# aliftffd/ViT-vs-Raw-IQ

Measured on AMD Instinct MI355X. Metric: IQ frames/sec training (fwd+loss+bwd+clip+AdamW), higher is better.
Workload: dtype bf16; 1 GPU; ViT-Tiny/16 224x224 C=1 19cls (BASELINE configs[1]); config_id=B, per_gpu_batch=256, global_batch=256, parallelism=dp1, hipgraph=True

## Files before the change

### include/iqvit.h

```cpp
#ifndef IQVIT_H
#define IQVIT_H
#include <stddef.h>
#include <stdint.h>

#ifdef __cplusplus
extern "C" {
#endif

typedef void* iq_stream_t;

enum { IQ_STATUS_OK = 0, IQ_STATUS_ARG = 1, IQ_STATUS_UNSUPPORTED = 2, IQ_STATUS_LAUNCH = 3 };

typedef struct iq_dropout {
  uint64_t seed;
  uint32_t step;
  uint32_t site;
  float p;
  const uint32_t* step_dev;
} iq_dropout_t;
#define IQ_SITE_IMPAIR 0xFFFFFFFFu
#define IQ_SITE_SYNTH 0xFFFFFFFEu

int iq_ln_supported(int D);
int iq_ln_fwd(const void* z, const float* gamma, const float* beta, void* x, float* mean, float* rstd, int M, int D,
              float eps, iq_stream_t stream);
size_t iq_ln_bwd_ws_bytes(int D);
int iq_ln_bwd(const void* dx, const void* z, const float* mean, const float* rstd, const float* gamma, void* dz,
              void* dy, const iq_dropout_t* drop, float* dgamma, float* dbeta, float* ws, int accumulate, int M,
              int D, iq_stream_t stream);
int iq_ln_bwd_partial_rows(int M, int D);

typedef struct iq_epilogue {
  const float* bias;
  int relu;
  const float* pe;
  int tok, seq, cls_off;
  iq_dropout_t drop;
  const void* gate;
  int ldg;
  float gate_scale;
  const void* residual;
  int ldr;
} iq_epilogue_t;
int iq_gemm_bf16_nt(const void* A, int lda, const void* B, int ldb, void* C, int ldc, int M, int N, int K,
                    const iq_epilogue_t* epi, iq_stream_t stream);

int iq_gemm_ln_supported(int D, int K);
int iq_gemm_bf16_ln(const void* A, int lda, const void* W, int ldw, const float* bias, const void* residual, int ldr,
                    const iq_dropout_t* drop, const float* gamma, const float* beta, float eps, void* Z, void* X,
                    float* mean, float* rstd, int M, int D, int K, iq_stream_t stream);

int iq_gemm_lnbwd_supported(int D, int K);
int iq_gemm_lnbwd_partial_rows(int M);
int iq_gemm_bf16_lnbwd(const void* A, int lda, const void* Wt, int ldw, const void* residual, int ldr, const void* z,
                       const float* mean, const float* rstd, const float* gamma, const iq_dropout_t* drop, void* dz,
                       void* dy, float* partial, int M, int D, int K, iq_stream_t stream);

int iq_ffn_chain_supported(int S, int D, int F);
int iq_ffn_chain_bwd_partial_rows(int M);
size_t iq_ffn_chain_gate_bytes(int M, int F);
int iq_ffn_chain_bwd(const void* dO, const void* W2t, const void* gate_bits, float gate_scale, void* gH, const void* W1t,
                     const void* residual, const void* z1, const float* mean, const float* rstd, const float* gamma,
                     const iq_dropout_t* drop, void* dz, void* dy, float* partial, const void* Wot, void* dA, int frames, int S,
                     int D, int F, iq_stream_t stream);
int iq_qkv_dgrad_ffn_chain_bwd(const void* gQKV, const void* Wqkv_t, const void* residual0, const void* z2, const float* mean2,
                               const float* rstd2, const float* gamma2, const iq_dropout_t* drop2, void* dz2, void* dy2, float* partial2,
                               const void* W2t, const void* gate_bits, float gate_scale, void* gH, const void* W1t, const void* residual,
                               const void* z1, const float* mean, const float* rstd, const float* gamma, const iq_dropout_t* drop, void* dz,
                               void* dy, float* partial, const void* Wot, void* dA, int frames, int S, int D, int F, iq_stream_t stream);
int iq_ffn_chain_fwd(const void* X1, const void* W1, const float* b1, const iq_dropout_t* drop1, void* H, const void* W2,
                     const float* b2, const iq_dropout_t* drop2, const float* gamma, const float* beta, float eps, void* Z,
                     void* X, float* mean, float* rstd, void* gate_bits, int frames, int S, int D, int F, iq_stream_t stream);
int iq_attn_out_ffn_chain_fwd(const void* A, const void* Wo, const float* bo, const iq_dropout_t* drop0, const void* R,
                              const float* gamma1, const float* beta1, void* Z1, void* X1, float* mean1, float* rstd1,
                              const void* W1, const float* b1, const iq_dropout_t* drop1, void* H, const void* W2, const float* b2,
                              const iq_dropout_t* drop2, const float* gamma2, const float* beta2, float eps, void* Z2, void* X,
                              float* mean2, float* rstd2, void* gate_bits, const void* Wq, const float* bq, void* Yq, int frames,
                              int S, int D, int F, iq_stream_t stream);

size_t iq_wgrad_ws_bytes(int M, int N, int K);
int iq_gemm_bf16_wgrad(const void* dY, int ldy, const void* X, int ldx, float* dW, float* dbias, int M, int N, int K,
                       float* ws, size_t ws_bytes, int accumulate, iq_stream_t stream);

typedef struct iq_wgrad_problem {
  const void* dY;
  int ldy;
  const void* X;
  int ldx;
  float* dW;
  float* dbias;
  int N, K;
} iq_wgrad_problem_t;
typedef struct iq_reduce_seg {
  const float* partials;
  int rows;
  int64_t row_stride;
  float* out;
  int64_t n;
} iq_reduce_seg_t;
size_t iq_wgrad_grouped_ws_bytes(const iq_wgrad_problem_t* probs, int nprob, int M, int max_workgroups);
int iq_gemm_bf16_wgrad_grouped(const iq_wgrad_problem_t* probs, int nprob, int M, float* ws, size_t ws_bytes,
                               int accumulate, int max_workgroups, const iq_reduce_seg_t* extra, int nextra,
                               iq_stream_t stream);

int iq_attn_supported(int S, int dh);
int iq_attn_fwd(const void* qkv, void* out, float* lse, int B, int S, int H, int dh, iq_stream_t stream);
int iq_attn_bwd(const void* qkv, const void* out, const void* dout, const float* lse, void* dqkv, int B, int S, int H,
                int dh, iq_stream_t stream);
int iq_attn_fwd_masked(const void* qkv, void* out, float* lse, const uint8_t* mask, long mask_hstride, int B, int S,
                       int H, int dh, iq_stream_t stream);
int iq_attn_bwd_masked(const void* qkv, const void* out, const void* dout, const float* lse, void* dqkv,
                       const uint8_t* mask, long mask_hstride, int B, int S, int H, int dh, iq_stream_t stream);
int iq_attn_probs(const void* qkv, const float* lse, float* out, long out_bstride, int B, int S, int H, int dh,
                  int rows, int heads, iq_stream_t stream);
int iq_attn_grad_probs(const void* qkv, const float* lse, const void* dout, float* out, long out_bstride, int B, int S,
                       int H, int dh, int rows, int heads, int positive, iq_stream_t stream);
int iq_attn_relevance_step(const void* qkv, const float* lse, const void* dout, const float* r_in, float* r_out, int B,
                           int S, int H, int dh, iq_stream_t stream);

int iq_frames_preprocess(const float* raw, float* out, int n_frames, int len, int take, const float* stats,
                         iq_stream_t stream);
typedef struct iq_impair {
  float phase_lo, phase_hi;
  float cfo_lo, cfo_hi;
  int   rot90;
  int   conj;
  int   shift_max;
  float gain_db_lo, gain_db_hi;
  float snr_db_lo, snr_db_hi;
  uint64_t seed; uint32_t step;
  uint64_t frame_base;
} iq_impair_t;
int iq_frames_impair(const float* raw, float* out, float* drawn, int n_frames, int len, int take, const float* stats,
                     const iq_impair_t* imp, iq_stream_t stream);
#define IQ_SYNTH_MAX_CLASSES 128
#define IQ_SYNTH_MAX_SNRS 64
typedef struct iq_synth_class { int kind; int offset; int count; } iq_synth_class_t;
typedef struct iq_synth {
  const float* points;
  const iq_synth_class_t* classes; int n_classes;
  const float* snrs_db; int n_snrs;
  int balanced;
  uint64_t seed; uint32_t stream;
  uint64_t frame_base;
} iq_synth_t;
int iq_frames_synth(float* raw , int64_t* labels, float* snr ,
                    float* drawn ,
                    int32_t* symbols , int n_frames, int len, const iq_synth_t* par, iq_stream_t stream);
typedef struct iq_waveform {
  const float* points; const iq_synth_class_t* classes; int n_classes;
  const float* snrs_db; int n_snrs; int balanced;
  uint64_t seed; uint32_t stream; uint64_t frame_base;
  int sps;
  int span;
  int n_phase;
  int timing;
  const float* pulse;
  const int32_t* fpulse;
  int n_taps;
  float los;
  float tap_sigma[8];
} iq_waveform_t;
int iq_frames_waveform(float* raw , int64_t* labels, float* snr, float* drawn ,
                       int32_t* symbols , float* taps , int n_frames, int len,
                       const iq_waveform_t* par, iq_stream_t stream);
enum { IQ_RX_GIVEN = 0, IQ_RX_OERDER_MEYR = 1, IQ_RX_ENERGY = 2 };
typedef struct iq_receiver {
  int sps;
  int span;
  int n_frac;
  int mode;
  int normalise;
  const float* table;
  const int32_t* u;
} iq_receiver_t;
int iq_frames_receive(const float* raw , float* sym , float* est ,
                      float* energy , int n_frames, int len, const iq_receiver_t* par, iq_stream_t stream);
int iq_frames_receive_bwd(const float* dsym , const float* sym, const float* est, float* dx ,
                          int n_frames, int len, const iq_receiver_t* par, iq_stream_t stream);
typedef struct iq_spectrogram {
  int n_fft;
  int hop;
  int pad;
  int width;
  int mode;
  float inv_norm, floor, scale, shift;
} iq_spectrogram_t;
int iq_frames_spectrogram(const float* x , const float* table ,
                          float* out , int n_frames, int len, const iq_spectrogram_t* par,
                          iq_stream_t stream);
int iq_frames_spectrogram_bwd(const float* x, const float* table, const float* dout ,
                              float* dx , int n_frames, int len, const iq_spectrogram_t* par,
                              iq_stream_t stream);
typedef struct iq_cyclic {
  int n_fft;
  int hop;
  int pad;
  int columns;
  int kind;
  int mode;
  float inv_norm, floor, scale, shift;
} iq_cyclic_t;
int iq_frames_cyclic(const float* x , const float* table , const float* rot ,
                     float* out , int n_frames, int len, const iq_cyclic_t* par, iq_stream_t stream);
int iq_patchify(const float* src, void* patches, int kind, int B, int C, int H, int W, int p, int Kpad,
                iq_stream_t stream);
int iq_cls_rows(const float* cls, const float* pe, void* x0, int B, int S, int D, const iq_dropout_t* drop,
                iq_stream_t stream);
int iq_embed_bwd_gather(const void* dx0, void* demb, float* dcls, int B, int S, int tok, int D, int has_cls,
                        const iq_dropout_t* drop, int accumulate, iq_stream_t stream);
int iq_embed_dgrad(const void* demb, const void* w_bf16, int Kpad, float* dsrc, int kind, int B, int C, int H, int W, int p,
                   int D, iq_stream_t stream);
int iq_linf_step(float* x_adv, const float* grad, const float* x0, float alpha, float eps, float lo, float hi, size_t n,
                 iq_stream_t stream);

int iq_head_fwd(const void* x, const float* ln_g, const float* ln_b, const float* W, const float* b, float* featn,
                float* hstat, float* logits, int B, int S, int D, int K, int pool, iq_stream_t stream);
int iq_ce_fwd_bwd(const float* logits, const int64_t* labels, int B, int K, float smoothing, float denom,
                  float* loss_sum, int32_t* n_correct, float* dlogits, iq_stream_t stream);
int iq_head_bwd(const float* dlogits, const float* featn, const float* hstat, const float* ln_g, const float* ln_b,
                const float* W, float* dW, float* db, float* dln_g, float* dln_b, void* dx, int B, int S, int D, int K,
                int pool, int accumulate, iq_stream_t stream);

size_t iq_gradnorm_ws_bytes(size_t n);
int iq_gradnorm_sq(const float* g, size_t n, float grad_scale, float* ws, float* out, iq_stream_t stream);
int iq_adamw_step(float* p, const float* g, float* m, float* v, void* shadow_bf16, size_t n, float lr, float beta1,
                  float beta2, float eps, float weight_decay, int step, const float* gnorm_sq, float max_norm,
                  float grad_scale, const float* dyn, iq_stream_t stream);
int iq_counter_add(uint32_t* ctr_u32, uint32_t inc_u32, float* ctr_f32, float inc_f32, iq_stream_t stream);
int iq_cast_bf16(const float* src, void* dst, size_t n, iq_stream_t stream);
int iq_transpose_cast_bf16(const float* src, void* dst, int rows, int cols, iq_stream_t stream);

typedef struct iq_model_cfg {
  int kind;
  int in_channels;
  int img_h, img_w, patch;
  int seq_length, conv_k, use_cls;
  int num_classes, d_model, n_head, n_layers, ffn_hidden;
  float drop_prob;
} iq_model_cfg_t;

typedef struct iq_model iq_model_t;

int iq_model_create(const iq_model_cfg_t* cfg, iq_model_t** out);
void iq_model_destroy(iq_model_t* m);
const char* iq_model_last_error(const iq_model_t* m);
int iq_model_tokens(const iq_model_t* m);
size_t iq_model_param_floats(const iq_model_t* m);
int iq_model_param_entries(const iq_model_t* m);
int iq_model_param_entry(const iq_model_t* m, int i, char* name, int name_cap, size_t* offset, int* ndim, int* dims);
size_t iq_model_shadow_bytes(const iq_model_t* m);
size_t iq_model_workspace_bytes(const iq_model_t* m, int batch, int training);
int iq_model_bind(iq_model_t* m, float* params, float* grads, const float* pe, void* shadow);
int iq_model_bind_step_counter(iq_model_t* m, uint32_t* counter);
int iq_model_refresh_shadow(iq_model_t* m, iq_stream_t stream);
int iq_model_refresh_transposed(iq_model_t* m, iq_stream_t stream);
int iq_model_forward(iq_model_t* m, const float* src, int batch, void* workspace, size_t ws_bytes, int training,
                     uint64_t seed, uint32_t step, float* enc_out, float* logits, iq_stream_t stream);
int iq_model_backward(iq_model_t* m, const float* dlogits, const float* denc, int batch, void* workspace,
                      size_t ws_bytes, int accumulate, int stage_hi, int stage_lo, iq_stream_t stream);
int iq_model_grad_range(const iq_model_t* m, int stage_hi, int stage_lo, size_t* off, size_t* len);
#define IQ_BWD_PARAM_GRADS 1
int iq_model_backward_input(iq_model_t* m, const float* dlogits, const float* denc, int batch, void* workspace,
                            size_t ws_bytes, float* dsrc, int flags, iq_stream_t stream);
int iq_model_attention(iq_model_t* m, const void* workspace, size_t ws_bytes, int batch, int layer, int rows,
                       int heads, float* out, long out_bstride, iq_stream_t stream);
int iq_model_attention_rollout(iq_model_t* m, const void* workspace, size_t ws_bytes, int batch, float alpha,
                               float* out, iq_stream_t stream);
int iq_model_attention_relevance(iq_model_t* m, const float* dlogits, int batch, void* workspace, size_t ws_bytes,
                                 float* rel, float* const* maps, int rows, int heads, int positive, long out_bstride,
                                 iq_stream_t stream);

#define IQ_PROF_FAMILIES 8
int iq_prof_enable(int on);
int iq_prof_collect(double* ms, long long* count);
size_t iq_prof_kernels(char* out, size_t cap, int reset);

#ifdef __cplusplus
}
#endif
#endif
```

### vit-vs-raw-iq_amd/_native.py

```python
from __future__ import annotations

import ctypes as C
import os

_HERE = os.path.dirname(os.path.abspath(__file__))
LIB_PATH = os.environ.get("IQ_LIBIQVIT") or os.path.join(_HERE, "libiqvit.so")

BWD_PARAM_GRADS = 1

STATUS = {0: "ok", 1: "invalid argument", 2: "unsupported shape/configuration", 3: "HIP launch error"}


class IqError(RuntimeError):
    pass


class Dropout(C.Structure):
    _fields_ = [("seed", C.c_uint64), ("step", C.c_uint32), ("site", C.c_uint32), ("p", C.c_float),
                ("step_dev", C.c_void_p)]


class Impair(C.Structure):
    _fields_ = [("phase_lo", C.c_float), ("phase_hi", C.c_float), ("cfo_lo", C.c_float), ("cfo_hi", C.c_float),
                ("rot90", C.c_int), ("conj", C.c_int), ("shift_max", C.c_int), ("gain_db_lo", C.c_float),
                ("gain_db_hi", C.c_float), ("snr_db_lo", C.c_float), ("snr_db_hi", C.c_float), ("seed", C.c_uint64),
                ("step", C.c_uint32), ("frame_base", C.c_uint64)]


class SynthClass(C.Structure):
    _fields_ = [("kind", C.c_int), ("offset", C.c_int), ("count", C.c_int)]


class Synth(C.Structure):
    _fields_ = [("points", C.c_void_p), ("classes", C.POINTER(SynthClass)), ("n_classes", C.c_int),
                ("snrs_db", C.POINTER(C.c_float)), ("n_snrs", C.c_int), ("balanced", C.c_int), ("seed", C.c_uint64),
                ("stream", C.c_uint32), ("frame_base", C.c_uint64)]


class Waveform(C.Structure):
    _fields_ = [("points", C.c_void_p), ("classes", C.POINTER(SynthClass)), ("n_classes", C.c_int),
                ("snrs_db", C.POINTER(C.c_float)), ("n_snrs", C.c_int), ("balanced", C.c_int), ("seed", C.c_uint64),
                ("stream", C.c_uint32), ("frame_base", C.c_uint64), ("sps", C.c_int), ("span", C.c_int), ("n_phase", C.c_int),
                ("timing", C.c_int), ("pulse", C.c_void_p), ("fpulse", C.c_void_p), ("n_taps", C.c_int), ("los", C.c_float),
                ("tap_sigma", C.c_float * 8)]


class Receiver(C.Structure):
    _fields_ = [("sps", C.c_int), ("span", C.c_int), ("n_frac", C.c_int), ("mode", C.c_int), ("normalise", C.c_int),
                ("table", C.c_void_p), ("u", C.c_void_p)]


class Spectrogram(C.Structure):
    _fields_ = [("n_fft", C.c_int), ("hop", C.c_int), ("pad", C.c_int), ("width", C.c_int), ("mode", C.c_int),
                ("inv_norm", C.c_float), ("floor", C.c_float), ("scale", C.c_float), ("shift", C.c_float)]


class Cyclic(C.Structure):
    _fields_ = [("n_fft", C.c_int), ("hop", C.c_int), ("pad", C.c_int), ("columns", C.c_int), ("kind", C.c_int),
                ("mode", C.c_int), ("inv_norm", C.c_float), ("floor", C.c_float), ("scale", C.c_float), ("shift", C.c_float)]


class Epilogue(C.Structure):
    _fields_ = [("bias", C.c_void_p), ("relu", C.c_int), ("pe", C.c_void_p), ("tok", C.c_int), ("seq", C.c_int),
                ("cls_off", C.c_int), ("drop", Dropout), ("gate", C.c_void_p), ("ldg", C.c_int),
                ("gate_scale", C.c_float), ("residual", C.c_void_p), ("ldr", C.c_int)]


class WgradProblem(C.Structure):
    _fields_ = [("dY", C.c_void_p), ("ldy", C.c_int), ("X", C.c_void_p), ("ldx", C.c_int), ("dW", C.c_void_p),
                ("dbias", C.c_void_p), ("N", C.c_int), ("K", C.c_int)]


class ReduceSeg(C.Structure):
    _fields_ = [("partials", C.c_void_p), ("rows", C.c_int), ("row_stride", C.c_int64), ("out", C.c_void_p),
                ("n", C.c_int64)]


class ModelCfg(C.Structure):
    _fields_ = [("kind", C.c_int), ("in_channels", C.c_int), ("img_h", C.c_int), ("img_w", C.c_int),
                ("patch", C.c_int), ("seq_length", C.c_int), ("conv_k", C.c_int), ("use_cls", C.c_int),
                ("num_classes", C.c_int), ("d_model", C.c_int), ("n_head", C.c_int), ("n_layers", C.c_int),
                ("ffn_hidden", C.c_int), ("drop_prob", C.c_float)]


_P, _I, _Z, _F = C.c_void_p, C.c_int, C.c_size_t, C.c_float
_U64, _U32 = C.c_uint64, C.c_uint32

SIGNATURES = {
    "iq_ln_supported": (_I, [_I]),
    "iq_ln_fwd": (_I, [_P, _P, _P, _P, _P, _P, _I, _I, _F, _P]),
    "iq_ln_bwd_ws_bytes": (_Z, [_I]),
    "iq_ln_bwd_partial_rows": (_I, [_I, _I]),
    "iq_ln_bwd": (_I, [_P, _P, _P, _P, _P, _P, _P, C.POINTER(Dropout), _P, _P, _P, _I, _I, _I, _P]),
    "iq_gemm_bf16_nt": (_I, [_P, _I, _P, _I, _P, _I, _I, _I, _I, C.POINTER(Epilogue), _P]),
    "iq_gemm_ln_supported": (_I, [_I, _I]),
    "iq_gemm_bf16_ln": (_I, [_P, _I, _P, _I, _P, _P, _I, C.POINTER(Dropout), _P, _P, _F, _P, _P, _P, _P, _I, _I, _I, _P]),
    "iq_gemm_lnbwd_supported": (_I, [_I, _I]),
    "iq_gemm_lnbwd_partial_rows": (_I, [_I]),
    "iq_gemm_bf16_lnbwd": (_I, [_P, _I, _P, _I, _P, _I, _P, _P, _P, _P, C.POINTER(Dropout), _P, _P, _P, _I, _I, _I, _P]),
    "iq_ffn_chain_supported": (_I, [_I, _I, _I]),
    "iq_ffn_chain_bwd_partial_rows": (_I, [_I]),
    "iq_ffn_chain_bwd": (_I, [_P, _P, _P, _F, _P, _P, _P, _P, _P, _P, _P, C.POINTER(Dropout), _P, _P, _P, _P, _P, _I, _I, _I, _I, _P]),
    "iq_qkv_dgrad_ffn_chain_bwd": (_I, [_P, _P, _P, _P, _P, _P, _P, C.POINTER(Dropout), _P, _P, _P,
                                        _P, _P, _F, _P, _P, _P, _P, _P, _P, _P, C.POINTER(Dropout), _P, _P, _P, _P, _P, _I, _I, _I, _I, _P]),
    "iq_ffn_chain_gate_bytes": (_Z, [_I, _I]),
    "iq_ffn_chain_fwd": (_I, [_P, _P, _P, C.POINTER(Dropout), _P, _P, _P, C.POINTER(Dropout), _P, _P, _F, _P, _P, _P, _P, _P, _I, _I,
                              _I, _I, _P]),
    "iq_attn_out_ffn_chain_fwd": (_I, [_P, _P, _P, C.POINTER(Dropout), _P, _P, _P, _P, _P, _P, _P,
                                       _P, _P, C.POINTER(Dropout), _P, _P, _P, C.POINTER(Dropout), _P, _P, _F, _P, _P, _P, _P, _P,
                                       _P, _P, _P, _I, _I, _I, _I, _P]),
    "iq_wgrad_ws_bytes": (_Z, [_I, _I, _I]),
    "iq_gemm_bf16_wgrad": (_I, [_P, _I, _P, _I, _P, _P, _I, _I, _I, _P, _Z, _I, _P]),
    "iq_wgrad_grouped_ws_bytes": (_Z, [_P, _I, _I, _I]),
    "iq_gemm_bf16_wgrad_grouped": (_I, [_P, _I, _I, _P, _Z, _I, _I, _P, _I, _P]),
    "iq_attn_supported": (_I, [_I, _I]),
    "iq_attn_fwd": (_I, [_P, _P, _P, _I, _I, _I, _I, _P]),
    "iq_attn_bwd": (_I, [_P, _P, _P, _P, _P, _I, _I, _I, _I, _P]),
    "iq_attn_fwd_masked": (_I, [_P, _P, _P, _P, C.c_long, _I, _I, _I, _I, _P]),
    "iq_attn_bwd_masked": (_I, [_P, _P, _P, _P, _P, _P, C.c_long, _I, _I, _I, _I, _P]),
    "iq_attn_probs": (_I, [_P, _P, _P, C.c_long, _I, _I, _I, _I, _I, _I, _P]),
    "iq_attn_grad_probs": (_I, [_P, _P, _P, _P, C.c_long, _I, _I, _I, _I, _I, _I, _I, _P]),
    "iq_attn_relevance_step": (_I, [_P, _P, _P, _P, _P, _I, _I, _I, _I, _P]),
    "iq_frames_preprocess": (_I, [_P, _P, _I, _I, _I, C.POINTER(C.c_float), _P]),
    "iq_frames_impair": (_I, [_P, _P, _P, _I, _I, _I, C.POINTER(C.c_float), C.POINTER(Impair), _P]),
    "iq_frames_synth": (_I, [_P, _P, _P, _P, _P, _I, _I, C.POINTER(Synth), _P]),
    "iq_frames_waveform": (_I, [_P, _P, _P, _P, _P, _P, _I, _I, C.POINTER(Waveform), _P]),
    "iq_frames_receive": (_I, [_P, _P, _P, _P, _I, _I, C.POINTER(Receiver), _P]),
    "iq_frames_receive_bwd": (_I, [_P, _P, _P, _P, _I, _I, C.POINTER(Receiver), _P]),
    "iq_frames_spectrogram": (_I, [_P, _P, _P, _I, _I, C.POINTER(Spectrogram), _P]),
    "iq_frames_spectrogram_bwd": (_I, [_P, _P, _P, _P, _I, _I, C.POINTER(Spectrogram), _P]),
    "iq_frames_cyclic": (_I, [_P, _P, _P, _P, _I, _I, C.POINTER(Cyclic), _P]),
    "iq_patchify": (_I, [_P, _P, _I, _I, _I, _I, _I, _I, _I, _P]),
    "iq_cls_rows": (_I, [_P, _P, _P, _I, _I, _I, C.POINTER(Dropout), _P]),
    "iq_embed_bwd_gather": (_I, [_P, _P, _P, _I, _I, _I, _I, _I, C.POINTER(Dropout), _I, _P]),
    "iq_embed_dgrad": (_I, [_P, _P, _I, _P, _I, _I, _I, _I, _I, _I, _I, _P]),
    "iq_linf_step": (_I, [_P, _P, _P, _F, _F, _F, _F, _Z, _P]),
    "iq_head_fwd": (_I, [_P, _P, _P, _P, _P, _P, _P, _P, _I, _I, _I, _I, _I, _P]),
    "iq_ce_fwd_bwd": (_I, [_P, _P, _I, _I, _F, _F, _P, _P, _P, _P]),
    "iq_head_bwd": (_I, [_P, _P, _P, _P, _P, _P, _P, _P, _P, _P, _P, _I, _I, _I, _I, _I, _I, _P]),
    "iq_gradnorm_ws_bytes": (_Z, [_Z]),
    "iq_gradnorm_sq": (_I, [_P, _Z, _F, _P, _P, _P]),
    "iq_adamw_step": (_I, [_P, _P, _P, _P, _P, _Z, _F, _F, _F, _F, _F, _I, _P, _F, _F, _P, _P]),
    "iq_counter_add": (_I, [_P, _U32, _P, _F, _P]),
    "iq_cast_bf16": (_I, [_P, _P, _Z, _P]),
    "iq_transpose_cast_bf16": (_I, [_P, _P, _I, _I, _P]),
    "iq_model_create": (_I, [C.POINTER(ModelCfg), C.POINTER(_P)]),
    "iq_model_destroy": (None, [_P]),
    "iq_model_last_error": (C.c_char_p, [_P]),
    "iq_model_tokens": (_I, [_P]),
    "iq_model_param_floats": (_Z, [_P]),
    "iq_model_param_entries": (_I, [_P]),
    "iq_model_param_entry": (_I, [_P, _I, C.c_char_p, _I, C.POINTER(_Z), C.POINTER(_I), C.POINTER(_I)]),
    "iq_model_shadow_bytes": (_Z, [_P]),
    "iq_model_workspace_bytes": (_Z, [_P, _I, _I]),
    "iq_model_bind": (_I, [_P, _P, _P, _P, _P]),
    "iq_model_bind_step_counter": (_I, [_P, _P]),
    "iq_model_refresh_shadow": (_I, [_P, _P]),
    "iq_model_refresh_transposed": (_I, [_P, _P]),
    "iq_model_forward": (_I, [_P, _P, _I, _P, _Z, _I, _U64, _U32, _P, _P, _P]),
    "iq_model_backward": (_I, [_P, _P, _P, _I, _P, _Z, _I, _I, _I, _P]),
    "iq_model_grad_range": (_I, [_P, _I, _I, C.POINTER(_Z), C.POINTER(_Z)]),
    "iq_model_backward_input": (_I, [_P, _P, _P, _I, _P, _Z, _P, _I, _P]),
    "iq_model_attention": (_I, [_P, _P, _Z, _I, _I, _I, _I, _P, C.c_long, _P]),
    "iq_model_attention_rollout": (_I, [_P, _P, _Z, _I, _F, _P, _P]),
    "iq_model_attention_relevance": (_I, [_P, _P, _I, _P, _Z, _P, C.POINTER(_P), _I, _I, _I, C.c_long, _P]),
    "iq_prof_enable": (_I, [_I]),
    "iq_prof_collect": (_I, [C.POINTER(C.c_double), C.POINTER(C.c_longlong)]),
    "iq_prof_kernels": (_Z, [C.c_char_p, _Z, _I]),
}

_lib = None


def lib():
    global _lib
    if _lib is None:
        if not os.path.exists(LIB_PATH):
            raise IqError(
                f"{LIB_PATH} not found: the HIP extension is not built. Run "
                "`python -c 'import __graft_entry__ as g; g.build()'` (or `make -C vit-vs-raw-iq_amd/csrc`). "
                "There is no CPU fallback.")
        L = C.CDLL(LIB_PATH)
        for name, (res, args) in SIGNATURES.items():
            fn = getattr(L, name)
            fn.restype = res
            fn.argtypes = args
        _lib = L
    return _lib


def check(rc, what, model=None):
    if rc != 0:
        detail = ""
        if model is not None:
            msg = lib().iq_model_last_error(model)
            if msg:
                detail = ": " + msg.decode()
        raise IqError(f"{what} failed: {STATUS.get(rc, rc)}{detail}")


def ptr(t):
    return None if t is None else t.data_ptr()


def stream_handle():
    import torch
    return torch.cuda.current_stream().cuda_stream
```

### vit-vs-raw-iq_amd/csrc/gemm_lnbwd.hip

```cpp

#include "common.h"
#include "gemm_common.h"
#include "gemm_ring.h"
#include "iqvit.h"
#include "prof.h"

namespace {

constexpr int LB_THREADS = 256;

struct LnBwdParams {
  const bf16* A; const bf16* B; const bf16* residual;
  int lda, ldb, ldr, M, K;
  const bf16* Z; const float* mean; const float* rstd; const float* gamma;
  bf16* dZ; bf16* dY;
  float* partial;
  int drop_on; IqRng rng; uint32_t thresh; float dscale;
};

template <int BMT, int BN>
__global__ __launch_bounds__(LB_THREADS, 2) void gemm_lnbwd_kernel(const LnBwdParams p) {
  using Ring = RingShape<BMT, BN>;
  constexpr int BK2 = Ring::BK2, NS = Ring::NS, STAGE_BYTES = Ring::STAGE_BYTES, WN = Ring::WN, NT = Ring::NT, NP = NT / 2, MT = Ring::MT;
  constexpr int A_LD = Ring::A_LD, B_LD = Ring::B_LD, PER_STAGE = Ring::PER_STAGE, NRS = Ring::NRS;
  constexpr int TAIL_LOADS = (BMT / (4 * (64 / ((BN == 192) ? 8 : 16)))) * (BN / (8 * ((BN == 192) ? 8 : 16)));
  constexpr int N = BN;
  static_assert(NRS >= 2, "tile shape");
  extern __shared__ __attribute__((aligned(16))) unsigned char smem[];

  const int tid = threadIdx.x, lane = tid & 63, wave = tid >> 6;
  const int wm = wave >> 1, wn = wave & 1;
  const int g = lane >> 4, c16 = lane & 15;
  const bool odd = (g & 1) != 0;
  const int m0 = blockIdx.x * BMT;

  f32x4 acc[MT][NT];
#pragma unroll
  for (int i = 0; i < MT; ++i)
#pragma unroll
    for (int j = 0; j < NT; ++j) acc[i][j] = f32x4{0.f, 0.f, 0.f, 0.f};

  const int prow = lane >> 2, pch = lane & 3;
  const bf16* a_src[A_LD];
  const bf16* r_src[A_LD];
  const bf16* b_src[B_LD];
#pragma unroll
  for (int i = 0; i < A_LD; ++i) {
    const int row = (wave * A_LD + i) * 16 + prow;
    const int gm = min(m0 + row, p.M - 1);
    a_src[i] = p.A + (long)gm * p.lda + (pch ^ ring_swz64(row)) * 8;
    r_src[i] = p.residual + (long)gm * p.ldr + (pch ^ ring_swz64(row)) * 8;
  }
#pragma unroll
  for (int i = 0; i < B_LD; ++i) {
    const int row = (wave * B_LD + i) * 16 + prow;
    b_src[i] = p.B + (long)row * p.ldb + (pch ^ ring_swz64(row)) * 8;
  }
  const int nk = p.K / BK2;
  bf16x8 idf[2];
#pragma unroll
  for (int h = 0; h < 2; ++h) {
    const int estar = 16 * h + (lane & 15) - 8 * (lane >> 4);
#pragma unroll
    for (int e = 0; e < 8; ++e) idf[h][e] = (bf16)(e == estar ? 1.0f : 0.0f);
  }
  auto issue = [&](int ks) {
    unsigned char* st = smem + (ks % NS) * STAGE_BYTES;
    if (ks >= nk) {
#pragma unroll
      for (int i = 0; i < A_LD; ++i)
        __builtin_amdgcn_global_load_lds((gbl_cvoid_t*)(r_src[i] + (ks - nk) * BK2), (lds_void_t*)(st + (wave * A_LD + i) * 1024), 16, 0, 0);
      return;
    }
#pragma unroll
    for (int i = 0; i < A_LD; ++i)
      __builtin_amdgcn_global_load_lds((gbl_cvoid_t*)(a_src[i] + ks * BK2), (lds_void_t*)(st + (wave * A_LD + i) * 1024), 16, 0, 0);
#pragma unroll
    for (int i = 0; i < B_LD; ++i)
      __builtin_amdgcn_global_load_lds((gbl_cvoid_t*)(b_src[i] + ks * BK2),
                                       (lds_void_t*)(st + BMT * BK2 * 2 + (wave * B_LD + i) * 1024), 16, 0, 0);
  };

  constexpr int LPR = (BN == 192) ? 8 : 16, NV = BN / (8 * LPR);
  constexpr int RPW = 64 / LPR, RPB = 4 * RPW, ITER = BMT / RPB;
  constexpr int LDI = BN + 8;
  static_assert(BMT * LDI * 2 <= NS * STAGE_BYTES && RPB * 2 * BN * 4 <= NS * STAGE_BYTES, "the tail's LDS fits in the ring");
  const int lj = lane % LPR, rsub = lane / LPR;
  bf16x8 zr[ITER][NV];
  auto issue_tail = [&]() {
#pragma unroll
    for (int it = 0; it < ITER; ++it) {
      const int gm = min(m0 + it * RPB + wave * RPW + rsub, p.M - 1);
#pragma unroll
      for (int v = 0; v < NV; ++v) zr[it][v] = *reinterpret_cast<const bf16x8*>(p.Z + (long)gm * N + (v * LPR + lj) * 8);
    }
  };

  const IqRng rng = p.drop_on ? rng_resolve(p.rng) : p.rng;
  float* side = reinterpret_cast<float*>(smem + NS * STAGE_BYTES);
  const int sr = tid & (BMT - 1);
  const int sgm = min(m0 + sr, p.M - 1);
  float side_v = 0.f;
  if (tid < 2 * BMT) side_v = tid < BMT ? p.mean[sgm] : p.rstd[sgm];
  f32x4 side_g = {0.f, 0.f, 0.f, 0.f};
  if (tid < N / 4) side_g = *reinterpret_cast<const f32x4*>(p.gamma + tid * 4);
  {
    const int d = ring_phase() * 2;
    for (int i = 0; i < d; ++i) __builtin_amdgcn_s_sleep(8);
  }
  issue(0);
  issue(1);
  if (tid < 2 * BMT) side[tid] = side_v;
  if (tid < N / 4) *reinterpret_cast<f32x4*>(side + 2 * BMT + tid * 4) = side_g;
  const int ch = lane >> 4;
  for (int ks = 0; ks < nk; ++ks) {
    if (ks + 1 < nk) wait_vmcnt<PER_STAGE>();
    else wait_vmcnt<A_LD>();
    ring_barrier();
    issue(ks + 2);
    const bf16* As = reinterpret_cast<const bf16*>(smem + (ks % NS) * STAGE_BYTES);
    const bf16* Bs = As + BMT * BK2;
    bf16x8 af[MT], bfr[NT];
#pragma unroll
    for (int i = 0; i < MT; ++i) {
      const int row = wm * (BMT / 2) + i * 16 + (lane & 15);
      af[i] = *reinterpret_cast<const bf16x8*>(As + row * BK2 + (ch ^ ring_swz64(row)) * 8);
    }
#pragma unroll
    for (int j = 0; j < NT; ++j) {
      const int row = wn * WN + j * 16 + (lane & 15);
      bfr[j] = *reinterpret_cast<const bf16x8*>(Bs + row * BK2 + (ch ^ ring_swz64(row)) * 8);
    }
#pragma unroll
    for (int i = 0; i < MT; ++i)
#pragma unroll
      for (int j = 0; j < NT; ++j)
        acc[i][j] = __builtin_amdgcn_mfma_f32_16x16x32_bf16(bfr[j], af[i], acc[i][j], 0, 0, 0);
  }
  auto residual_stage = [&](auto tc) {
    constexpr int t = decltype(tc)::value;
    const bf16* As = reinterpret_cast<const bf16*>(smem + ((nk + t) % NS) * STAGE_BYTES);
    if (wn == (2 * t) / NT) {
      bf16x8 af[MT];
#pragma unroll
      for (int i = 0; i < MT; ++i) {
        const int row = wm * (BMT / 2) + i * 16 + (lane & 15);
        af[i] = *reinterpret_cast<const bf16x8*>(As + row * BK2 + (ch ^ ring_swz64(row)) * 8);
      }
#pragma unroll
      for (int h = 0; h < 2; ++h) {
        constexpr int jbase = (2 * t) % NT;
#pragma unroll
        for (int i = 0; i < MT; ++i)
          acc[i][jbase + h] = __builtin_amdgcn_mfma_f32_16x16x32_bf16(idf[h], af[i], acc[i][jbase + h], 0, 0, 0);
      }
    }
  };
  static_for<NRS>([&](auto tc) {
    constexpr int t = decltype(tc)::value;
    if constexpr (t + 2 < NRS) {
      wait_barrier<A_LD>();
      issue(nk + t + 2);
    } else if constexpr (t + 2 == NRS) {
      wait_barrier<A_LD>();
      issue_tail();
      asm volatile("" ::: "memory");
    } else {
      wait_barrier<TAIL_LOADS>();
    }
    residual_stage(tc);
  });

  bf16* img = reinterpret_cast<bf16*>(smem);
  const int row0l = wm * (BMT / 2), col0 = wn * WN;
  __builtin_amdgcn_s_barrier();
  asm volatile("" ::: "memory");
#pragma unroll
  for (int i = 0; i < MT; ++i) {
#pragma unroll
    for (int jp = 0; jp < NP; ++jp) {
      float w[8];
#pragma unroll
      for (int r = 0; r < 4; ++r) {
        const float va = acc[i][2 * jp][r], vb = acc[i][2 * jp + 1][r];
        const auto sw = __builtin_amdgcn_permlane16_swap(__float_as_uint(va), __float_as_uint(vb), false, false);
        w[r] = __uint_as_float(sw[0]);
        w[4 + r] = __uint_as_float(sw[1]);
      }
      const int col = col0 + (odd ? (2 * jp + 1) * 16 + 4 * (g - 1) : (2 * jp) * 16 + 4 * g);
      *reinterpret_cast<bf16x8*>(img + (row0l + i * 16 + c16) * LDI + col) = pack8(w);
    }
  }
  asm volatile("s_waitcnt lgkmcnt(0)" ::: "memory");
  __builtin_amdgcn_s_barrier();
  asm volatile("" ::: "memory");
  float gmm[NV][8], ag[NV][8], ab[NV][8];
#pragma unroll
  for (int v = 0; v < NV; ++v) {
    const f32x4 a = *reinterpret_cast<const f32x4*>(side + 2 * BMT + (v * LPR + lj) * 8);
    const f32x4 b = *reinterpret_cast<const f32x4*>(side + 2 * BMT + (v * LPR + lj) * 8 + 4);
#pragma unroll
    for (int e = 0; e < 4; ++e) { gmm[v][e] = a[e]; gmm[v][4 + e] = b[e]; }
#pragma unroll
    for (int e = 0; e < 8; ++e) { ag[v][e] = 0.f; ab[v][e] = 0.f; }
  }
  const float invD = 1.0f / (float)N;
#pragma unroll
  for (int it = 0; it < ITER; ++it) {
    const int rl = it * RPB + wave * RPW + rsub;
    const long row = (long)m0 + rl;
    const bool ok = row < p.M;
    const float mean = side[rl], rstd = side[BMT + rl];
    float xh[NV][8], dy[NV][8];
    float s1 = 0.f, s2 = 0.f;
#pragma unroll
    for (int v = 0; v < NV; ++v) {
      bf16x8 td = *reinterpret_cast<const bf16x8*>(img + rl * LDI + (v * LPR + lj) * 8);
      bf16x8 tz = zr[it][v];
      if (!ok) { td = bf16x8{}; tz = bf16x8{}; }
      unpack8(tz, xh[v]);
      unpack8(td, dy[v]);
#pragma unroll
      for (int e = 0; e < 8; ++e) {
        xh[v][e] = ok ? (xh[v][e] - mean) * rstd : 0.f;
        ag[v][e] += dy[v][e] * xh[v][e];
        ab[v][e] += dy[v][e];
        dy[v][e] *= gmm[v][e];
        s1 += dy[v][e];
        s2 += dy[v][e] * xh[v][e];
      }
    }
#pragma unroll
    for (int o = LPR / 2; o > 0; o >>= 1) { s1 += __shfl_xor(s1, o, 64); s2 += __shfl_xor(s2, o, 64); }
    const float c1 = s1 * invD, c2 = s2 * invD;
    if (ok) {
#pragma unroll
      for (int v = 0; v < NV; ++v) {
        float o[8];
#pragma unroll
        for (int e = 0; e < 8; ++e) o[e] = rstd * (dy[v][e] - c1 - xh[v][e] * c2);
        const long off = row * N + (v * LPR + lj) * 8;
        *reinterpret_cast<bf16x8*>(p.dZ + off) = pack8(o);
        if (p.drop_on) {
          const uint32_t keep = dropout_keep8(rng, (uint64_t)off >> 3, p.thresh);
#pragma unroll
          for (int e = 0; e < 8; ++e) o[e] = ((keep >> e) & 1u) ? o[e] * p.dscale : 0.f;
          *reinterpret_cast<bf16x8*>(p.dY + off) = pack8(o);
        }
      }
    }
  }
  float* red = reinterpret_cast<float*>(smem);
  asm volatile("s_waitcnt lgkmcnt(0)" ::: "memory");
  __builtin_amdgcn_s_barrier();
  asm volatile("" ::: "memory");
  const int rslot = wave * RPW + rsub;
#pragma unroll
  for (int v = 0; v < NV; ++v) {
    const int c = (v * LPR + lj) * 8;
#pragma unroll
    for (int e = 0; e < 8; ++e) {
      red[rslot * 2 * N + c + e] = ag[v][e];
      red[rslot * 2 * N + N + c + e] = ab[v][e];
    }
  }
  asm volatile("s_waitcnt lgkmcnt(0)" ::: "memory");
  __builtin_amdgcn_s_barrier();
  asm volatile("" ::: "memory");
  for (int c = tid; c < 2 * N; c += LB_THREADS) {
    float sum = 0.f;
    for (int r = 0; r < RPB; ++r) sum += red[r * 2 * N + c];
    p.partial[(long)blockIdx.x * 2 * N + c] = sum;
  }
}

template <int BMT, int BN>
int launch(const LnBwdParams& p, hipStream_t st) {
  const size_t lds = RingShape<BMT, BN>::BYTES + (2 * BMT + BN) * sizeof(float);
  auto k = gemm_lnbwd_kernel<BMT, BN>;
  if (lds > 48 * 1024) (void)hipFuncSetAttribute((const void*)k, hipFuncAttributeMaxDynamicSharedMemorySize, (int)lds);
  k<<<(p.M + BMT - 1) / BMT, LB_THREADS, lds, st>>>(p);
  return iq_launch_status();
}

inline int lnbwd_block_rows(int M) { return (M + 127) / 128 <= 320 ? 64 : 128; }

}

extern "C" int iq_gemm_lnbwd_supported(int D, int K) { return ((D == 128 || D == 192) && K >= 64 && K % 32 == 0) ? 1 : 0; }
extern "C" int iq_gemm_lnbwd_partial_rows(int M) {
  if (M <= 0) return 0;
  const int r = lnbwd_block_rows(M);
  return (M + r - 1) / r;
}

extern "C" int iq_gemm_bf16_lnbwd(const void* A, int lda, const void* Wt, int ldw, const void* residual, int ldr,
                                  const void* z, const float* mean, const float* rstd, const float* gamma,
                                  const iq_dropout_t* drop, void* dz, void* dy, float* partial, int M, int D, int K,
                                  iq_stream_t stream) {
  if (M <= 0) return IQ_OK;
  if (!A || !Wt || !residual || !z || !mean || !rstd || !gamma || !dz || !partial) return IQ_ERR_ARG;
  if (!iq_gemm_lnbwd_supported(D, K) || (lda % 8) || (ldw % 8) || (ldr % 8)) return IQ_ERR_UNSUPPORTED;
  if (((uintptr_t)A | (uintptr_t)Wt | (uintptr_t)residual | (uintptr_t)z | (uintptr_t)dz | (uintptr_t)dy | (uintptr_t)gamma) % 16)
    return IQ_ERR_ARG;
  LnBwdParams p = {};
  p.A = (const bf16*)A; p.B = (const bf16*)Wt; p.residual = (const bf16*)residual;
  p.lda = lda; p.ldb = ldw; p.ldr = ldr; p.M = M; p.K = K;
  p.Z = (const bf16*)z; p.mean = mean; p.rstd = rstd; p.gamma = gamma;
  p.dZ = (bf16*)dz; p.dY = (bf16*)dy; p.partial = partial;
  if (!dropout_unpack(drop, &p.drop_on, &p.rng, &p.thresh, &p.dscale) || (p.drop_on && !dy)) return IQ_ERR_ARG;
  hipStream_t st = (hipStream_t)stream;
  IQ_PROF(IQ_FAM_GEMM_NT, st);
  IQ_PROF_K(2.0 * ((double)M * K + (double)D * K + (double)M * D * (3 + (p.drop_on ? 1 : 0))) + 8.0 * M, 2.0 * (double)M * D * K,
            "gemm_lnbwd_kernel<%d, %d>", lnbwd_block_rows(M), D);
  if (lnbwd_block_rows(M) == 64) return D == 192 ? launch<64, 192>(p, st) : launch<64, 128>(p, st);
  return D == 192 ? launch<128, 192>(p, st) : launch<128, 128>(p, st);
}
```

### vit-vs-raw-iq_amd/csrc/gemm_wgrad.hip

```cpp
#include "common.h"
#include <stdlib.h>
#include <string.h>
#include "iqvit.h"
#include "prof.h"

#include "gemm_wgrad_big.h"

namespace {

constexpr int WG_THREADS = 512;
constexpr int TN = 128;
constexpr int YLD = TN + 16;

struct WgradParams {
  const bf16* Y; const bf16* X;
  int ldy, ldx, M, N, K;
  float* slab;
  float* bslab;
  int tiles_n, tiles_k, splits, rows_per_split;
#ifdef IQ_WGRAD_STAMPS
  unsigned long long* stamps;
#endif
};

#ifdef IQ_WGRAD_STAMPS
#define IQ_WTICK(i) do { asm volatile("s_memtime %0\n\ts_waitcnt lgkmcnt(0)" : "=s"(tn_) :: "memory"); tk_[i] += tn_ - tl_; tl_ = tn_; } while (0)
#else
#define IQ_WTICK(i) do {} while (0)
#endif

__device__ __forceinline__ bf16x8 tr_frag(const bf16* tile, int ld, int r0, int c0, int lane) {
  const int i16 = lane & 15, g = lane >> 4;
  const bf16* a = tile + (r0 + 4 * g + (i16 >> 2)) * ld + c0 + 4 * (i16 & 3);
  typedef __attribute__((address_space(3))) s16x4 lds_s16x4;
  s16x4 lo = __builtin_amdgcn_ds_read_tr16_b64_v4i16((lds_s16x4*)(a));
  s16x4 hi = __builtin_amdgcn_ds_read_tr16_b64_v4i16((lds_s16x4*)(a + 16 * ld));
  s16x8 v = {lo[0], lo[1], lo[2], lo[3], hi[0], hi[1], hi[2], hi[3]};
  return __builtin_bit_cast(bf16x8, v);
}

template <int TK, int MC>
__global__ __launch_bounds__(WG_THREADS, 4) void wgrad_kernel(const WgradParams p) {
  constexpr int XLD = TK + 16;
  constexpr int KT = TK / 64;
  constexpr int Y_CH = MC * (TN / 8) / WG_THREADS;
  constexpr int X_CH = MC * (TK / 8) / WG_THREADS;
  extern __shared__ __attribute__((aligned(16))) unsigned char smem[];
  bf16* Ys = reinterpret_cast<bf16*>(smem);
  bf16* Xs = Ys + MC * YLD;

  const int tid = threadIdx.x, lane = tid & 63, wave = tid >> 6;
  const int wn = wave >> 2, wk = wave & 3;
  const int ntile = p.tiles_n * p.tiles_k;
  const int lid = xcd_remap(blockIdx.x, gridDim.x);
  const int split = lid / ntile, tile = lid % ntile;
  const int n0 = (tile / p.tiles_k) * TN, k0 = (tile % p.tiles_k) * TK;
  const int mbeg = split * p.rows_per_split;
  const int mend = min(p.M, mbeg + p.rows_per_split);
  const bool do_bias = p.bslab != nullptr && (tile % p.tiles_k) == 0 && wk == 0;

  f32x4 acc[4][KT], accb[4];
#pragma unroll
  for (int i = 0; i < 4; ++i) {
    accb[i] = f32x4{0.f, 0.f, 0.f, 0.f};
#pragma unroll
    for (int j = 0; j < KT; ++j) acc[i][j] = f32x4{0.f, 0.f, 0.f, 0.f};
  }
  bf16x8 ones;
#pragma unroll
  for (int e = 0; e < 8; ++e) ones[e] = (bf16)1.0f;

  bf16x8 ry[Y_CH], rx[X_CH];
  auto gload = [&](int mb) {
#pragma unroll
    for (int c = 0; c < Y_CH; ++c) {
      const int id = tid + c * WG_THREADS, row = id / (TN / 8), ch = id % (TN / 8);
      const int gm = mb + row, gn = n0 + ch * 8;
      bf16x8 v = {};
      if (gm < mend && gn < p.N) v = *reinterpret_cast<const bf16x8*>(p.Y + (long)gm * p.ldy + gn);
      ry[c] = v;
    }
#pragma unroll
    for (int c = 0; c < X_CH; ++c) {
      const int id = tid + c * WG_THREADS, row = id / (TK / 8), ch = id % (TK / 8);
      const int gm = mb + row, gk = k0 + ch * 8;
      bf16x8 v = {};
      if (gm < mend && gk < p.K) v = *reinterpret_cast<const bf16x8*>(p.X + (long)gm * p.ldx + gk);
      rx[c] = v;
    }
  };
  auto lstore = [&]() {
#pragma unroll
    for (int c = 0; c < Y_CH; ++c) {
      const int id = tid + c * WG_THREADS, row = id / (TN / 8), ch = id % (TN / 8);
      *reinterpret_cast<bf16x8*>(Ys + row * YLD + ch * 8) = ry[c];
    }
#pragma unroll
    for (int c = 0; c < X_CH; ++c) {
      const int id = tid + c * WG_THREADS, row = id / (TK / 8), ch = id % (TK / 8);
      *reinterpret_cast<bf16x8*>(Xs + row * XLD + ch * 8) = rx[c];
    }
  };

#ifdef IQ_WGRAD_STAMPS
  unsigned long long tk_[6] = {0, 0, 0, 0, 0, 0}, tl_, tn_;
  asm volatile("s_memtime %0\n\ts_waitcnt lgkmcnt(0)" : "=s"(tl_) :: "memory");
#endif
  if (mbeg < mend) {
    gload(mbeg);
    lstore();
  }
  __syncthreads();
  IQ_WTICK(0);
  for (int mb = mbeg; mb < mend; mb += MC) {
    const bool more = mb + MC < mend;
    if (more) gload(mb + MC);
    IQ_WTICK(1);
#pragma unroll
    for (int s = 0; s < MC / 32; ++s) {
      bf16x8 af[4], bfr[KT];
#pragma unroll
      for (int i = 0; i < 4; ++i) af[i] = tr_frag(Ys, YLD, s * 32, wn * 64 + i * 16, lane);
#pragma unroll
      for (int j = 0; j < KT; ++j) bfr[j] = tr_frag(Xs, XLD, s * 32, wk * (TK / 4) + j * 16, lane);
#pragma unroll
      for (int i = 0; i < 4; ++i) {
#pragma unroll
        for (int j = 0; j < KT; ++j)
          acc[i][j] = __builtin_amdgcn_mfma_f32_16x16x32_bf16(af[i], bfr[j], acc[i][j], 0, 0, 0);
        if (do_bias) accb[i] = __builtin_amdgcn_mfma_f32_16x16x32_bf16(af[i], ones, accb[i], 0, 0, 0);
      }
    }
    IQ_WTICK(2);
    __syncthreads();
    IQ_WTICK(3);
    if (more) {
#ifdef IQ_WGRAD_STAMPS
      asm volatile("s_waitcnt vmcnt(0)" ::: "memory");
      IQ_WTICK(4);
#endif
      lstore();
      __syncthreads();
      IQ_WTICK(5);
    }
  }
#ifdef IQ_WGRAD_STAMPS
  if (tid == 0 && p.stamps)
    for (int i = 0; i < 6; ++i) p.stamps[(long)blockIdx.x * 6 + i] = tk_[i];
#endif

  float* out = p.slab + (long)split * p.N * p.K;
#pragma unroll
  for (int i = 0; i < 4; ++i) {
#pragma unroll
    for (int r = 0; r < 4; ++r) {
      const int n = n0 + wn * 64 + i * 16 + (lane >> 4) * 4 + r;
      if (n < p.N) {
#pragma unroll
        for (int j = 0; j < KT; ++j) {
          const int k = k0 + wk * (TK / 4) + j * 16 + (lane & 15);
          if (k < p.K) out[(long)n * p.K + k] = acc[i][j][r];
        }
        if (do_bias && (lane & 15) == 0) p.bslab[(long)split * p.N + n] = accb[i][r];
      }
    }
  }
}

constexpr int PW_THREADS = 256, PW_T = 64, PW_ROWS = 32;
constexpr int PW_MAXW = 128;
constexpr int pw_ld(int t) { return t + 16; }
constexpr int PW_WAVE_LDS = PW_ROWS * (pw_ld(PW_MAXW) + pw_ld(PW_T));
constexpr int PW_RED_ROWS = 16;

constexpr int PW_MAXP = 4;
struct PwProb {
  const bf16* Y; const bf16* X;
  float* slab;
  float* bslab;
  int ldy, ldx, N, K, tiles_n, tiles_k, tile0;
  int tn, tk;
};
struct PwGroup {
  PwProb pr[PW_MAXP];
  int nprob, M, ntile, splits, rows_per_split;
#ifdef IQ_WGRAD_STAMPS
  unsigned long long* stamps;
#endif
};

template <int TN, int TK>
__device__ __forceinline__ void pw_body(const PwGroup& g, const PwProb& p, int tile, int split, unsigned char* smem) {
  constexpr int NI = TN / 16, NJ = TK / 16;
  constexpr int LDY = pw_ld(TN), LDX = pw_ld(TK);
  constexpr int YC = TN / 64, XC = TK / 64;
  constexpr int RED_LD = TK + 4;
  const int tid = threadIdx.x, lane = tid & 63;
  const int wave = __builtin_amdgcn_readfirstlane(tid >> 6);
  bf16* Ys = reinterpret_cast<bf16*>(smem) + wave * PW_WAVE_LDS;
  bf16* Xs = Ys + PW_ROWS * LDY;
  int nt, kt;
  if (p.tiles_n >= p.tiles_k) { nt = tile / p.tiles_k; kt = tile % p.tiles_k; }
  else { kt = tile / p.tiles_n; nt = tile % p.tiles_n; }
  const int n0 = nt * TN, k0 = kt * TK;
  const int mbeg = split * g.rows_per_split;
  const int mend = min(g.M, mbeg + g.rows_per_split);
  const bool do_bias = p.bslab != nullptr && kt == 0;

  f32x4 acc[NI][NJ];
#pragma unroll
  for (int i = 0; i < NI; ++i)
#pragma unroll
    for (int j = 0; j < NJ; ++j) acc[i][j] = f32x4{0.f, 0.f, 0.f, 0.f};
  float bs[YC][8];
#pragma unroll
  for (int c = 0; c < YC; ++c)
#pragma unroll
    for (int e = 0; e < 8; ++e) bs[c][e] = 0.f;

  const int prow = ((lane >> 4) & 3) + ((lane >> 3) & 1) * 4, pch = lane & 7;
  const bf16* yptr[YC];
  const bf16* xptr[XC];
#pragma unroll
  for (int c = 0; c < YC; ++c) { const int col = n0 + c * 64 + pch * 8; yptr[c] = p.Y + (long)prow * p.ldy + (col < p.N ? col : 0); }
#pragma unroll
  for (int c = 0; c < XC; ++c) { const int col = k0 + c * 64 + pch * 8; xptr[c] = p.X + (long)prow * p.ldx + (col < p.K ? col : 0); }
  const long ystep = 8L * p.ldy, xstep = 8L * p.ldx;
  bf16x8 ry[YC][4], rx[XC][4];
  auto gload = [&](int m0) {
    const bool full = m0 + PW_ROWS <= mend;
#pragma unroll
    for (int j = 0; j < 4; ++j) {
      const bool ok = full || (m0 + j * 8 + prow < mend);
#pragma unroll
      for (int c = 0; c < YC; ++c) {
        bf16x8 v = {};
        if (ok) v = *reinterpret_cast<const bf16x8*>(yptr[c] + (long)m0 * p.ldy + j * ystep);
        ry[c][j] = v;
      }
#pragma unroll
      for (int c = 0; c < XC; ++c) {
        bf16x8 v = {};
        if (ok) v = *reinterpret_cast<const bf16x8*>(xptr[c] + (long)m0 * p.ldx + j * xstep);
        rx[c][j] = v;
      }
    }
  };
  auto lstore = [&]() {
    if (do_bias) {
#pragma unroll
      for (int c = 0; c < YC; ++c)
#pragma unroll
        for (int j = 0; j < 4; ++j)
#pragma unroll
          for (int e = 0; e < 8; ++e) bs[c][e] += (float)ry[c][j][e];
    }
#pragma unroll
    for (int j = 0; j < 4; ++j) {
#pragma unroll
      for (int c = 0; c < YC; ++c) *reinterpret_cast<bf16x8*>(Ys + (j * 8 + prow) * LDY + c * 64 + pch * 8) = ry[c][j];
#pragma unroll
      for (int c = 0; c < XC; ++c) *reinterpret_cast<bf16x8*>(Xs + (j * 8 + prow) * LDX + c * 64 + pch * 8) = rx[c][j];
    }
  };

  int m = mbeg + wave * PW_ROWS, mnext = m + 4 * PW_ROWS;
  if (m < mend) {
    gload(m);
    lstore();
    if (mnext < mend) gload(mnext);
  }
  while (m < mend) {
    asm volatile("" ::: "memory");
    __builtin_amdgcn_wave_barrier();
    bf16x8 af[NI], bfr[NJ];
#pragma unroll
    for (int i = 0; i < NI; ++i) af[i] = tr_frag(Ys, LDY, 0, i * 16, lane);
#pragma unroll
    for (int j = 0; j < NJ; ++j) bfr[j] = tr_frag(Xs, LDX, 0, j * 16, lane);
    asm volatile("s_waitcnt lgkmcnt(0)" ::: "memory");
    __builtin_amdgcn_wave_barrier();
#pragma unroll
    for (int i = 0; i < NI; ++i)
#pragma unroll
      for (int j = 0; j < NJ; ++j)
        acc[i][j] = __builtin_amdgcn_mfma_f32_16x16x32_bf16(af[i], bfr[j], acc[i][j], 0, 0, 0);
    m = mnext; mnext += 4 * PW_ROWS;
    if (m < mend) {
      lstore();
      if (mnext < mend) gload(mnext);
    }
  }

  float* red = reinterpret_cast<float*>(smem);
  float* out = p.slab + (long)split * p.N * p.K;
  static_assert(4 * PW_RED_ROWS * RED_LD * 4 <= 4 * PW_WAVE_LDS * 2, "the reduction area fits the stage areas");
#pragma unroll
  for (int h = 0; h < NI; ++h) {
    __syncthreads();
#pragma unroll
    for (int j = 0; j < NJ; ++j)
#pragma unroll
      for (int r = 0; r < 4; ++r)
        red[(wave * PW_RED_ROWS + (lane >> 4) * 4 + r) * RED_LD + j * 16 + (lane & 15)] = acc[h][j][r];
    __syncthreads();
    constexpr int F4 = PW_RED_ROWS * TK / 4;
#pragma unroll
    for (int c = 0; c < (F4 + PW_THREADS - 1) / PW_THREADS; ++c) {
      const int id = tid + c * PW_THREADS;
      if (id < F4) {
        const int row = id / (TK / 4), c4 = (id % (TK / 4)) * 4;
        f32x4 sum = *reinterpret_cast<const f32x4*>(red + row * RED_LD + c4);
#pragma unroll
        for (int w = 1; w < 4; ++w) sum += *reinterpret_cast<const f32x4*>(red + (w * PW_RED_ROWS + row) * RED_LD + c4);
        const int n = n0 + h * 16 + row, k = k0 + c4;
        if (n < p.N && k < p.K) *reinterpret_cast<f32x4*>(out + (long)n * p.K + k) = sum;
      }
    }
  }
  if (do_bias) {
    __syncthreads();
#pragma unroll
    for (int c = 0; c < YC; ++c)
#pragma unroll
      for (int e = 0; e < 8; ++e) {
        float v = bs[c][e];
        v += __shfl_xor(v, 8, 64);
        v += __shfl_xor(v, 16, 64);
        v += __shfl_xor(v, 32, 64);
        if (lane < 8) red[wave * TN + c * 64 + pch * 8 + e] = v;
      }
    __syncthreads();
    if (tid < TN && n0 + tid < p.N)
      p.bslab[(long)split * p.N + n0 + tid] = red[tid] + red[TN + tid] + red[2 * TN + tid] + red[3 * TN + tid];
  }
}

__global__ __launch_bounds__(PW_THREADS, 2) void wgrad_pw_kernel(const PwGroup g) {
  extern __shared__ __attribute__((aligned(16))) unsigned char smem[];
  const int lid = xcd_remap(blockIdx.x, gridDim.x);
  const int split = lid / g.ntile, gt = lid % g.ntile;
  PwProb p = g.pr[0];
#pragma unroll
  for (int i = 1; i < PW_MAXP; ++i)
    if (i < g.nprob && gt >= g.pr[i].tile0) p = g.pr[i];
  const int tile = gt - p.tile0;
  if (p.tn == 128) pw_body<128, 64>(g, p, tile, split, smem);
  else if (p.tk == 128) pw_body<64, 128>(g, p, tile, split, smem);
  else pw_body<64, 64>(g, p, tile, split, smem);
}

constexpr int RED_MAXX = 4;
struct RedSeg { const float* slab; float* out; long n, stride; int rows, blk0, tall; };
struct RedGroup { RedSeg s[2 * PW_MAXP + RED_MAXX]; int nseg, accumulate; };

inline int red_blocks(long n, int tall) { return (int)((n + (tall ? 63 : 255)) / (tall ? 64 : 256)); }

__global__ __launch_bounds__(256) void wgrad_reduce_kernel(const RedGroup g) {
  __shared__ f32x4 part[256];
  RedSeg sg = g.s[0];
#pragma unroll
  for (int i = 1; i < 2 * PW_MAXP + RED_MAXX; ++i)
    if (i < g.nseg && (int)blockIdx.x >= g.s[i].blk0) sg = g.s[i];
  const float* __restrict__ slab = sg.slab;
  float* __restrict__ out = sg.out;
  const long n = sg.n, stride = sg.stride;
  const long blk = (long)blockIdx.x - sg.blk0;
  const int rows = sg.rows, accumulate = g.accumulate;
  const int ncol = sg.tall ? 16 : 64, nsl = 256 / ncol;
  const int col = threadIdx.x % ncol, sl = threadIdx.x / ncol;
  const long i = (blk * ncol + col) * 4;
  f32x4 s = {0.f, 0.f, 0.f, 0.f};
  if (i + 4 <= n) {
#pragma unroll 8
    for (int sp = sl; sp < rows; sp += nsl) s += *reinterpret_cast<const f32x4*>(slab + (long)sp * stride + i);
  } else if (i < n) {
    for (int sp = sl; sp < rows; sp += nsl)
      for (int e = 0; e < 4 && i + e < n; ++e) s[e] += slab[(long)sp * stride + i + e];
  }
  part[sl * ncol + col] = s;
  __syncthreads();
  if (sl == 0 && i < n) {
    f32x4 t = part[col];
    for (int k = 1; k < nsl; ++k) t += part[k * ncol + col];
    if (i + 4 <= n) {
      f32x4* o = reinterpret_cast<f32x4*>(out + i);
      *o = accumulate ? *o + t : t;
    } else {
      for (int e = 0; e < 4 && i + e < n; ++e) out[i + e] = accumulate ? out[i + e] + t[e] : t[e];
    }
  }
}

struct WgradPlan { int tk, mc, tiles_n, tiles_k, splits, rows_per_split; };

inline WgradPlan wgrad_plan(int M, int N, int K) {
  WgradPlan w;
  w.tk = (K % 128 == 0 || K > 512) ? 128 : 64;
  w.mc = 64;
  const int MC = w.mc;
  w.tiles_n = (N + TN - 1) / TN;
  w.tiles_k = (K + w.tk - 1) / w.tk;
  const int tiles = w.tiles_n * w.tiles_k;
  int splits = 512 / tiles;
  const int max_splits = (M + 255) / 256;
  if (splits > max_splits) splits = max_splits;
  if (splits < 1) splits = 1;
  int rps = (M + splits - 1) / splits;
  rps = ((rps + MC - 1) / MC) * MC;
  w.rows_per_split = rps;
  w.splits = (M + rps - 1) / rps;
  return w;
}

inline bool pw_eligible(int N, int K) { return (long)N * K <= 512 * 1024; }
inline size_t pad4(size_t v) { return (v + 3) / 4 * 4; }

inline void pw_tile(int N, int K, int* tn, int* tk) {
  *tn = 64; *tk = 64;
  if (N >= K && N >= 256) *tn = 128;
  else if (K > N && K >= 256) *tk = 128;
}
struct PwPlan { int ntile, splits, rows_per_split; size_t floats; };
inline PwPlan pw_plan(const iq_wgrad_problem_t* pr, int nprob, int M, int max_wgs) {
  PwPlan w;
  w.ntile = 0;
  for (int i = 0; i < nprob; ++i) {
    int tn, tk;
    pw_tile(pr[i].N, pr[i].K, &tn, &tk);
    w.ntile += ((pr[i].N + tn - 1) / tn) * ((pr[i].K + tk - 1) / tk);
  }
  const int slots = (max_wgs > 0 && max_wgs < 512) ? max_wgs : 512;
  int splits = slots / w.ntile;
  const int max_splits = (M + 255) / 256;
  if (splits > max_splits) splits = max_splits;
  if (splits < 1) splits = 1;
  const int unit = 4 * PW_ROWS;
  int rps = (M + splits - 1) / splits;
  rps = ((rps + unit - 1) / unit) * unit;
  w.rows_per_split = rps;
  w.splits = (M + rps - 1) / rps;
  w.floats = 0;
  for (int i = 0; i < nprob; ++i) w.floats += (size_t)w.splits * (pad4((size_t)pr[i].N * pr[i].K) + pad4(pr[i].N));
  return w;
}
inline bool group_is_pw(const iq_wgrad_problem_t* pr, int nprob) {
  if (nprob < 1 || nprob > PW_MAXP) return false;
  for (int i = 0; i < nprob; ++i)
    if (!pw_eligible(pr[i].N, pr[i].K)) return false;
  return true;
}
inline size_t shared_ws_floats(int M, int N, int K) {
  const WgradPlan w = wgrad_plan(M, N, K);
  return (size_t)w.splits * (pad4((size_t)N * K) + pad4(N));
}

#ifdef IQ_WGRAD_STAMPS
unsigned long long* g_wstamps = nullptr;
#endif

int launch_reduce(const RedGroup& rg, int nblk, hipStream_t st) {
  IQ_PROF(IQ_FAM_WGRAD, st);
  wgrad_reduce_kernel<<<nblk, 256, 0, st>>>(rg);
  IQ_PROF_K(0.0, 0.0, "wgrad_reduce_kernel");
  return IQ_OK;
}

void wgrad_work(const iq_wgrad_problem_t* pr, int nprob, int M, double* bytes, double* flops) {
  *bytes = *flops = 0;
  for (int i = 0; i < nprob; ++i) {
    *bytes += 2.0 * M * ((double)pr[i].N + pr[i].K) + 4.0 * (double)pr[i].N * pr[i].K;
    *flops += 2.0 * M * (double)pr[i].N * pr[i].K;
  }
}

int wgrad_shared_one(const iq_wgrad_problem_t& pb, int M, float* ws, int accumulate, hipStream_t st) {
  const int N = pb.N, K = pb.K;
  const WgradPlan w = wgrad_plan(M, N, K);
  WgradParams q;
  q.Y = (const bf16*)pb.dY; q.X = (const bf16*)pb.X; q.ldy = pb.ldy; q.ldx = pb.ldx; q.M = M; q.N = N; q.K = K;
  q.slab = ws;
  q.bslab = pb.dbias ? ws + (size_t)w.splits * pad4((size_t)N * K) : nullptr;
  q.tiles_n = w.tiles_n; q.tiles_k = w.tiles_k; q.splits = w.splits; q.rows_per_split = w.rows_per_split;
#ifdef IQ_WGRAD_STAMPS
  q.stamps = g_wstamps;
#endif
  const int grid = w.tiles_n * w.tiles_k * w.splits;
  const size_t lds = (size_t)w.mc * (YLD + w.tk + 16) * 2;
  {
  IQ_PROF(IQ_FAM_WGRAD, st);
#define IQ_WG_LAUNCH(TK_, MC_)                                                                                   \
  do {                                                                                                           \
    auto k = wgrad_kernel<TK_, MC_>;                                                                             \
    if (lds > 48 * 1024) (void)hipFuncSetAttribute((const void*)k, hipFuncAttributeMaxDynamicSharedMemorySize, (int)lds); \
    k<<<grid, WG_THREADS, lds, st>>>(q);                                                                         \
  } while (0)
  if (w.tk == 128) IQ_WG_LAUNCH(128, 64);
  else IQ_WG_LAUNCH(64, 64);
#undef IQ_WG_LAUNCH
  double wbytes, wflops;
  wgrad_work(&pb, 1, M, &wbytes, &wflops);
  IQ_PROF_K(wbytes, wflops, "wgrad_kernel<%d, 64>", w.tk == 128 ? 128 : 64);
  }
  RedGroup rg;
  memset(&rg, 0, sizeof(rg));
  const long n = (long)N * K;
  rg.s[0] = RedSeg{q.slab, pb.dW, n, n, w.splits, 0, 0};
  int nblk = (int)((n + 255) / 256);
  rg.nseg = 1;
  if (pb.dbias) { rg.s[1] = RedSeg{q.bslab, pb.dbias, (long)N, (long)N, w.splits, nblk, 0}; nblk += (N + 255) / 256; rg.nseg = 2; }
  rg.accumulate = accumulate;
  return launch_reduce(rg, nblk, st);
}

}

#ifdef IQ_WGRAD_STAMPS
extern "C" void iq_debug_set_wgrad_stamps(unsigned long long* p) { g_wstamps = p; }
#endif

extern "C" size_t iq_wgrad_grouped_ws_bytes(const iq_wgrad_problem_t* probs, int nprob, int M, int max_workgroups) {
  if (!probs || nprob <= 0 || M <= 0) return 0;
  WbPlan wb;
  iq_wgrad_problem_t al[PW_MAXP];
  size_t big = 0;
  if (nprob <= PW_MAXP) {
    for (int i = 0; i < nprob; ++i) { al[i] = probs[i]; al[i].dY = nullptr; al[i].X = nullptr; al[i].ldy = 64; al[i].ldx = 64; }
    if (wgrad_big_plan(al, nprob, M, &wb)) big = wb.floats * sizeof(float);
  }
  if (group_is_pw(probs, nprob)) {
    const size_t b = pw_plan(probs, nprob, M, max_workgroups).floats * sizeof(float);
    return b > big ? b : big;
  }
  size_t mx = big / sizeof(float);
  for (int i = 0; i < nprob; ++i) {
    const size_t b = pw_eligible(probs[i].N, probs[i].K) ? pw_plan(probs + i, 1, M, max_workgroups).floats
                                                          : shared_ws_floats(M, probs[i].N, probs[i].K);
    if (b > mx) mx = b;
  }
  return mx * sizeof(float);
}

extern "C" int iq_gemm_bf16_wgrad_grouped(const iq_wgrad_problem_t* probs, int nprob, int M, float* ws, size_t ws_bytes,
                                          int accumulate, int max_workgroups, const iq_reduce_seg_t* extra, int nextra,
                                          iq_stream_t stream) {
  if (nextra < 0 || nextra > RED_MAXX || (nextra > 0 && !extra)) return IQ_ERR_ARG;
  for (int i = 0; i < nextra; ++i)
    if (!extra[i].partials || !extra[i].out || extra[i].rows <= 0 || extra[i].n <= 0 || extra[i].row_stride < extra[i].n ||
        (extra[i].row_stride % 4) || (((uintptr_t)extra[i].partials | (uintptr_t)extra[i].out) & 15))
      return IQ_ERR_ARG;
  auto add_extra = [&](RedGroup& rg, int& nblk) {
    for (int i = 0; i < nextra; ++i) {
      const int tall = extra[i].rows >= 64;
      rg.s[rg.nseg++] = RedSeg{extra[i].partials, extra[i].out, (long)extra[i].n, (long)extra[i].row_stride, extra[i].rows, nblk, tall};
      nblk += red_blocks(extra[i].n, tall);
    }
  };
  if (nprob <= 0 && nextra == 0) return IQ_OK;
  if (nprob > 0 && (!probs || !ws || M <= 0)) return IQ_ERR_ARG;
  for (int i = 0; i < nprob; ++i) {
    const iq_wgrad_problem_t& b = probs[i];
    if (b.N <= 0 || b.K <= 0 || !b.dY || !b.X || !b.dW) return IQ_ERR_ARG;
    if ((b.N % 8) || (b.K % 8) || (b.ldy % 8) || (b.ldx % 8)) return IQ_ERR_UNSUPPORTED;
    if (((uintptr_t)b.dW & 15) != 0) return IQ_ERR_ARG;
  }
  if (ws_bytes < iq_wgrad_grouped_ws_bytes(probs, nprob, M, max_workgroups)) return IQ_ERR_ARG;
  hipStream_t st = (hipStream_t)stream;
  double wbytes, wflops;
  wgrad_work(probs, nprob, M, &wbytes, &wflops);
  WbPlan wb;
  if (nprob > 0 && max_workgroups == 0 && wgrad_big_plan(probs, nprob, M, &wb) && ws_bytes >= wb.floats * sizeof(float)) {
    float *slab[PW_MAXP], *bslab[PW_MAXP];
    {
      IQ_PROF(IQ_FAM_WGRAD, st);
      wgrad_big_launch(probs, nprob, M, wb, ws, slab, bslab, st);
      IQ_PROF_K(wbytes, wflops, "wgrad_big_kernel<%d>", wb.tk);
    }
    RedGroup rg;
    memset(&rg, 0, sizeof(rg));
    int nblk = 0;
    for (int i = 0; i < nprob; ++i) {
      const long n = (long)probs[i].N * probs[i].K;
      rg.s[rg.nseg++] = RedSeg{slab[i], probs[i].dW, n, (long)pad4((size_t)n), wb.splits, nblk, 0};
      nblk += (int)((n + 255) / 256);
      if (probs[i].dbias) {
        rg.s[rg.nseg++] = RedSeg{bslab[i], probs[i].dbias, (long)probs[i].N, (long)pad4(probs[i].N), wb.splits, nblk, 0};
        nblk += (probs[i].N + 255) / 256;
      }
    }
    add_extra(rg, nblk);
    rg.accumulate = accumulate;
    launch_reduce(rg, nblk, st);
    return iq_launch_status();
  }
  if (!group_is_pw(probs, nprob)) {
    for (int i = 0; i < nprob; ++i) {
      int rc;
      if (pw_eligible(probs[i].N, probs[i].K)) {
        rc = iq_gemm_bf16_wgrad_grouped(probs + i, 1, M, ws, ws_bytes, accumulate, max_workgroups, nullptr, 0, stream);
      } else {
        rc = wgrad_shared_one(probs[i], M, ws, accumulate, st);
      }
      if (rc != IQ_OK) return rc;
    }
    if (nextra > 0) {
      RedGroup rg;
      memset(&rg, 0, sizeof(rg));
      int nblk = 0;
      add_extra(rg, nblk);
      rg.accumulate = accumulate;
      launch_reduce(rg, nblk, st);
    }
    return iq_launch_status();
  }
  const PwPlan w = pw_plan(probs, nprob, M, max_workgroups);
  PwGroup g;
  RedGroup rg;
  memset(&g, 0, sizeof(g));
  memset(&rg, 0, sizeof(rg));
  g.nprob = nprob; g.M = M; g.ntile = w.ntile; g.splits = w.splits; g.rows_per_split = w.rows_per_split;
#ifdef IQ_WGRAD_STAMPS
  g.stamps = g_wstamps;
#endif
  float* cur = ws;
  int tile0 = 0, nblk = 0;
  for (int i = 0; i < nprob; ++i) {
    const iq_wgrad_problem_t& b = probs[i];
    PwProb& q = g.pr[i];
    q.Y = (const bf16*)b.dY; q.X = (const bf16*)b.X; q.ldy = b.ldy; q.ldx = b.ldx; q.N = b.N; q.K = b.K;
    pw_tile(b.N, b.K, &q.tn, &q.tk);
    q.tiles_n = (b.N + q.tn - 1) / q.tn;
    q.tiles_k = (b.K + q.tk - 1) / q.tk;
    q.tile0 = tile0;
    tile0 += q.tiles_n * q.tiles_k;
    const long n = (long)b.N * b.K;
    q.slab = cur; cur += (size_t)w.splits * pad4((size_t)n);
    rg.s[rg.nseg++] = RedSeg{q.slab, b.dW, n, n, w.splits, nblk, 0};
    nblk += (int)((n + 255) / 256);
    if (b.dbias) {
      q.bslab = cur; cur += (size_t)w.splits * pad4(b.N);
      rg.s[rg.nseg++] = RedSeg{q.bslab, b.dbias, (long)b.N, (long)b.N, w.splits, nblk, 0};
      nblk += (b.N + 255) / 256;
    }
  }
  add_extra(rg, nblk);
  rg.accumulate = accumulate;
  const size_t lds_pw = (size_t)4 * PW_WAVE_LDS * 2;
  if (lds_pw > 48 * 1024) (void)hipFuncSetAttribute((const void*)wgrad_pw_kernel, hipFuncAttributeMaxDynamicSharedMemorySize, (int)lds_pw);
  {
    IQ_PROF(IQ_FAM_WGRAD, st);
    wgrad_pw_kernel<<<w.ntile * w.splits, PW_THREADS, lds_pw, st>>>(g);
    IQ_PROF_K(wbytes, wflops, "wgrad_pw_kernel");
  }
  launch_reduce(rg, nblk, st);
  return iq_launch_status();
}

extern "C" size_t iq_wgrad_ws_bytes(int M, int N, int K) {
  if (M <= 0 || N <= 0 || K <= 0) return 0;
  iq_wgrad_problem_t b;
  memset(&b, 0, sizeof(b));
  b.N = N; b.K = K;
  return iq_wgrad_grouped_ws_bytes(&b, 1, M, 0);
}

extern "C" int iq_gemm_bf16_wgrad(const void* dY, int ldy, const void* X, int ldx, float* dW, float* dbias, int M,
                                  int N, int K, float* ws, size_t ws_bytes, int accumulate, iq_stream_t stream) {
  if (N <= 0 || K <= 0) return IQ_OK;
  iq_wgrad_problem_t b;
  b.dY = dY; b.ldy = ldy; b.X = X; b.ldx = ldx; b.dW = dW; b.dbias = dbias; b.N = N; b.K = K;
  return iq_gemm_bf16_wgrad_grouped(&b, 1, M, ws, ws_bytes, accumulate, 0, nullptr, 0, stream);
}
```

### vit-vs-raw-iq_amd/csrc/model.hip

```cpp
#include <hip/hip_runtime.h>
#include <stdio.h>
#include <string.h>

#include <string>
#include <vector>

#include "attn_maps.h"
#include "common.h"
#include "iqvit.h"
#include "prof.h"

int head_bwd_dx_launch(const float* dlogits, const float* featn, const float* hstat, const float* ln_g, const float* W, void* dx,
                       int B, int S, int D, int K, int pool, hipStream_t st);
int embed_bwd_gather_launch(const void* dx0, void* demb, int B, int S, int tok, int D, int has_cls, const iq_dropout_t* drop,
                            hipStream_t st);

namespace {

struct Entry {
  std::string name;
  size_t off;
  int ndim;
  int dims[4];
};

struct LayerOff {
  size_t wqkv, bqkv, wo, bo, g1, be1, w1, b1, w2, b2, g2, be2, end;
  size_t t_wqkv, t_wo, t_w1, t_w2;
};

inline size_t align_up(size_t v, size_t a) { return (v + a - 1) / a * a; }

struct WsPlan {
  size_t step_ctr, patches, x0, head_feat, head_stat;
  struct L { size_t qkv, att, lse, z1, mean1, rstd1, x1, hid, gate, z2, mean2, rstd2, x2; };
  std::vector<L> layers;
  size_t gA, gB, gAtt, demb, wgrad_ws, wgrad_ws_bytes, ln_part[2], embw_scratch;
  size_t gZ, gY, gZ1, gY1, gH, gQKV;
  size_t total;
};

__global__ void bf16_to_f32_kernel(const bf16* __restrict__ s, float* __restrict__ d, size_t n8) {
  for (size_t i = (size_t)blockIdx.x * blockDim.x + threadIdx.x; i < n8; i += (size_t)gridDim.x * blockDim.x) {
    const bf16x8 v = reinterpret_cast<const bf16x8*>(s)[i];
    f32x4 a = {(float)v[0], (float)v[1], (float)v[2], (float)v[3]};
    f32x4 b = {(float)v[4], (float)v[5], (float)v[6], (float)v[7]};
    reinterpret_cast<f32x4*>(d)[2 * i] = a;
    reinterpret_cast<f32x4*>(d)[2 * i + 1] = b;
  }
}
__global__ void f32_into_bf16_kernel(const float* __restrict__ s, bf16* __restrict__ d, size_t n8, int add) {
  for (size_t i = (size_t)blockIdx.x * blockDim.x + threadIdx.x; i < n8; i += (size_t)gridDim.x * blockDim.x) {
    const f32x4 a = reinterpret_cast<const f32x4*>(s)[2 * i], b = reinterpret_cast<const f32x4*>(s)[2 * i + 1];
    float f[8] = {a[0], a[1], a[2], a[3], b[0], b[1], b[2], b[3]};
    if (add) {
      const bf16x8 o = reinterpret_cast<const bf16x8*>(d)[i];
#pragma unroll
      for (int e = 0; e < 8; ++e) f[e] += (float)o[e];
    }
    reinterpret_cast<bf16x8*>(d)[i] = pack8(f);
  }
}
__global__ void cast_pad_kernel(const float* __restrict__ s, bf16* __restrict__ d, int rows, int cols, int ld) {
  const long n = (long)rows * ld;
  for (long i = (long)blockIdx.x * blockDim.x + threadIdx.x; i < n; i += (long)gridDim.x * blockDim.x) {
    const int r = (int)(i / ld), c = (int)(i % ld);
    d[i] = (bf16)(c < cols ? s[(long)r * cols + c] : 0.f);
  }
}
__global__ void unpad_kernel(const float* __restrict__ s, float* __restrict__ d, int rows, int cols, int ld, int add) {
  const long n = (long)rows * cols;
  for (long i = (long)blockIdx.x * blockDim.x + threadIdx.x; i < n; i += (long)gridDim.x * blockDim.x) {
    const int r = (int)(i / cols), c = (int)(i % cols);
    const float v = s[(long)r * ld + c];
    d[i] = add ? d[i] + v : v;
  }
}
struct TransDesc { unsigned long long src_off, dst_off; int rows, cols, tile0, tiles_x; };
__global__ __launch_bounds__(256) void transpose_table_kernel(const float* __restrict__ params, unsigned char* __restrict__ shadow,
                                                              const TransDesc* __restrict__ tab, int nent) {
  __shared__ float t[32][33];
  int e = 0;
  while (e + 1 < nent && (int)blockIdx.x >= tab[e + 1].tile0) ++e;
  const TransDesc d = tab[e];
  const int local = blockIdx.x - d.tile0;
  const int bx = (local % d.tiles_x) * 32, by = (local / d.tiles_x) * 32;
  const float* src = params + d.src_off;
  bf16* dst = reinterpret_cast<bf16*>(shadow + d.dst_off);
  const int tx = threadIdx.x & 31, ty = threadIdx.x >> 5;
  for (int i = ty; i < 32; i += 8) {
    const int r = by + i, c = bx + tx;
    t[i][tx] = (r < d.rows && c < d.cols) ? src[(long)r * d.cols + c] : 0.f;
  }
  __syncthreads();
  for (int i = ty; i < 32; i += 8) {
    const int c = bx + i, r = by + tx;
    if (c < d.cols && r < d.rows) dst[(long)c * d.rows + r] = (bf16)t[tx][i];
  }
}

__global__ void rel_start_kernel(float* r, int n, int S, int cls) {
  for (int i = blockIdx.x * blockDim.x + threadIdx.x; i < n; i += gridDim.x * blockDim.x) {
    const int k = i % S;
    r[i] = cls ? (k == 0 ? 1.f : 0.f) : 1.0f / S;
  }
}

struct RelHook {
  float* const* maps;
  int rows, heads, positive;
  long bstride;
  float* rel;
  float* r[2];
};

__global__ void set_u32_kernel(uint32_t* p, uint32_t v, int bump) {
  if (threadIdx.x == 0 && blockIdx.x == 0) *p = bump ? *p + 1u : v;
}

inline int blocks_for(size_t n, int cap = 4096) {
  size_t b = (n + 255) / 256;
  if (b > (size_t)cap) b = cap;
  if (b < 1) b = 1;
  return (int)b;
}

}

struct iq_model {
  iq_model_cfg_t c;
  int S, tok, has_cls, P, Ppad, dh, pool, head_ln;
  std::vector<Entry> entries;
  size_t nparam;
  size_t emb_w, emb_b, cls, emb_end;
  std::vector<LayerOff> L;
  size_t hln_g, hln_b, head_w, head_b, head_begin;
  size_t sh_flat, sh_embw, sh_table, shadow_bytes;
  std::vector<TransDesc> ttab;
  int ttiles = 0;
  const void* table_uploaded_to = nullptr;
  float* params = nullptr;
  float* grads = nullptr;
  const float* pe = nullptr;
  unsigned char* shadow = nullptr;
  std::string err;
  uint32_t* step_ctr = nullptr;
  uint64_t last_seed = 0;
  bool last_tr = false;
  bool last_train_fwd = false;
  const void* fwd_ws = nullptr;
  int fwd_batch = 0;

  iq_dropout_t bwd_site(uint32_t id, const uint32_t* step_dev, bool tr) const {
    iq_dropout_t d;
    d.seed = last_seed; d.step = 0; d.site = id; d.p = tr ? c.drop_prob : 0.f; d.step_dev = step_dev;
    return d;
  }

  size_t add(const std::string& name, std::vector<int> dims, size_t& cur, bool aligned = true) {
    if (aligned) cur = align_up(cur, 64);
    Entry e;
    e.name = name; e.off = cur; e.ndim = (int)dims.size();
    size_t n = 1;
    for (int i = 0; i < 4; ++i) { e.dims[i] = i < e.ndim ? dims[i] : 1; n *= (size_t)e.dims[i]; }
    entries.push_back(e);
    cur += n;
    return e.off;
  }
  const bf16* sh(size_t off) const { return reinterpret_cast<const bf16*>(shadow + sh_flat) + off; }
  const bf16* sht(size_t byte_off) const { return reinterpret_cast<const bf16*>(shadow + byte_off); }
};

namespace {

int fail(iq_model* m, int code, const std::string& msg) {
  if (m) m->err = msg;
  return code;
}

WsPlan plan_ws(const iq_model* m, int B) {
  WsPlan w;
  const size_t D = m->c.d_model, F = m->c.ffn_hidden, S = m->S, H = m->c.n_head;
  const size_t M = (size_t)B * S, MT = (size_t)B * m->tok;
  size_t cur = 0;
  auto take = [&](size_t bytes) { size_t o = cur; cur = align_up(cur + bytes, 256); return o; };
  w.step_ctr = take(256);
  w.patches = take(MT * m->Ppad * 2);
  w.x0 = take(M * D * 2);
  w.head_feat = take((size_t)B * D * 4);
  w.head_stat = take((size_t)B * 2 * 4);
  w.layers.resize(m->c.n_layers);
  for (auto& l : w.layers) {
    l.qkv = take(M * 3 * D * 2);
    l.att = take(M * D * 2);
    l.lse = take((size_t)B * H * S * 4);
    l.z1 = take(M * D * 2);
    l.mean1 = take(M * 4);
    l.rstd1 = take(M * 4);
    l.x1 = take(M * D * 2);
    l.hid = take(M * F * 2);
    l.gate = take(iq_ffn_chain_gate_bytes((int)M, (int)F));
    l.z2 = take(M * D * 2);
    l.mean2 = take(M * 4);
    l.rstd2 = take(M * 4);
    l.x2 = take(M * D * 2);
  }
  w.gA = take(M * D * 2);
  w.gB = take(M * D * 2);
  w.gZ = take(M * D * 2);
  w.gY = take(M * D * 2);
  w.gZ1 = take(M * D * 2);
  w.gY1 = take(M * D * 2);
  w.gH = take(M * F * 2);
  w.gQKV = take(M * 3 * D * 2);
  w.gAtt = take(M * D * 2);
  w.demb = take(MT * D * 2);
  size_t wb = 0;
  auto mx = [&](size_t v) { if (v > wb) wb = v; };
  {
    iq_wgrad_problem_t g[4];
    memset(g, 0, sizeof(g));
    g[0].N = (int)D; g[0].K = (int)F;
    g[1].N = (int)F; g[1].K = (int)D;
    g[2].N = (int)D; g[2].K = (int)D;
    g[3].N = (int)(3 * D); g[3].K = (int)D;
    mx(iq_wgrad_grouped_ws_bytes(g, 4, (int)M, 0));
    for (int k = 0; k < 4; ++k) mx(iq_wgrad_grouped_ws_bytes(g + k, 1, (int)M, 0));
  }
  mx(iq_wgrad_ws_bytes((int)MT, (int)D, m->Ppad));
  w.wgrad_ws_bytes = wb;
  w.wgrad_ws = take(wb);
  size_t ln_rows_fused = (size_t)iq_gemm_lnbwd_partial_rows((int)M);
  if ((size_t)iq_ffn_chain_bwd_partial_rows((int)M) > ln_rows_fused) ln_rows_fused = (size_t)iq_ffn_chain_bwd_partial_rows((int)M);
  ln_rows_fused *= 2 * D * sizeof(float);
  const size_t ln_bytes = ln_rows_fused > iq_ln_bwd_ws_bytes((int)D) ? ln_rows_fused : iq_ln_bwd_ws_bytes((int)D);
  for (int k = 0; k < 2; ++k) w.ln_part[k] = take(ln_bytes);
  w.embw_scratch = take((size_t)D * m->Ppad * 4 + 256);
  w.total = cur;
  return w;
}

inline bool use_fused_ln(int D, int K) { return iq_gemm_ln_supported(D, K) && (D <= 192 || K <= 256); }

struct Route {
  bool chain;
  bool chain_takes_qkv_dgrad;
};
inline Route layer_route(int M, int S, int D, int F) {
  Route r;
  r.chain = iq_ffn_chain_supported(S, D, F) && M >= 8192;
  r.chain_takes_qkv_dgrad = r.chain && M <= 32768;
  return r;
}

#define IQ_TRY(expr, what)                                                              \
  do {                                                                                  \
    int rc_ = (expr);                                                                   \
    if (rc_ != IQ_OK) return fail(m, rc_, std::string(what) + " failed (status " + std::to_string(rc_) + ")"); \
  } while (0)

iq_dropout_t site(const iq_model* m, uint64_t seed, const uint32_t* step_dev, uint32_t id, bool training) {
  iq_dropout_t d;
  d.seed = seed; d.step = 0; d.site = id; d.p = training ? m->c.drop_prob : 0.f; d.step_dev = step_dev;
  return d;
}

}

extern "C" int iq_model_create(const iq_model_cfg_t* cfg, iq_model_t** out) {
  if (!cfg || !out) return IQ_ERR_ARG;
  *out = nullptr;
  iq_model* m = new iq_model();
  m->c = *cfg;
  const iq_model_cfg_t& c = m->c;
  auto bad = [&](const char* msg) { fprintf(stderr, "iq_model_create: %s\n", msg); delete m; return IQ_ERR_UNSUPPORTED; };
  if (c.d_model <= 0 || c.n_head <= 0 || c.n_layers < 0 || c.ffn_hidden <= 0 || c.num_classes <= 0 || c.in_channels <= 0)
    { delete m; return IQ_ERR_ARG; }
  if (c.d_model % c.n_head) return bad("d_model must be divisible by n_head");
  m->dh = c.d_model / c.n_head;
  if (m->dh != 16 && m->dh != 32 && m->dh != 64) return bad("head dim (d_model/n_head) must be 16, 32 or 64");
  if (c.ffn_hidden % 8) return bad("ffn_hidden must be a multiple of 8");
  if (!iq_ln_supported(c.d_model)) return bad("d_model not supported by the LayerNorm kernel");
  if (!(c.drop_prob >= 0.f && c.drop_prob < 1.f)) return bad("drop_prob must be in [0,1)");
  if (c.kind == 0) {
    if (c.patch <= 0 || c.img_h < c.patch || c.img_w < c.patch) return bad("bad image / patch size");
    m->tok = (c.img_h / c.patch) * (c.img_w / c.patch);
    m->has_cls = 1;
    m->P = c.in_channels * c.patch * c.patch;
    m->pool = 0;
    m->head_ln = 0;
  } else if (c.kind == 1) {
    if (c.conv_k <= 0 || c.seq_length < c.conv_k || (c.seq_length % c.conv_k)) return bad("bad seq_length / segment_size");
    m->tok = c.seq_length / c.conv_k;
    m->has_cls = c.use_cls ? 1 : 0;
    m->P = c.in_channels * c.conv_k;
    m->pool = m->has_cls ? 0 : 1;
    m->head_ln = 1;
  } else {
    delete m;
    return IQ_ERR_ARG;
  }
  m->S = m->tok + m->has_cls;
  m->Ppad = (int)align_up((size_t)m->P, 32);
  if (!iq_attn_supported(m->S, m->dh)) return bad("sequence too long for the attention backward kernel at this head dim");

  const int D = c.d_model, F = c.ffn_hidden, K = c.num_classes;
  size_t cur = 0;
  const std::string emb = c.kind == 0 ? "encoder.patch_embedding.projection" : "encoder.sequence_embedding.projection";
  if (c.kind == 0) m->emb_w = m->add(emb + ".weight", {D, c.in_channels, c.patch, c.patch}, cur);
  else m->emb_w = m->add(emb + ".weight", {D, c.in_channels, c.conv_k}, cur);
  m->emb_b = m->add(emb + ".bias", {D}, cur);
  m->cls = 0;
  if (m->has_cls) m->cls = m->add("encoder.cls_token", {1, 1, D}, cur);
  cur = align_up(cur, 64);
  m->emb_end = cur;
  m->L.resize(c.n_layers);
  for (int i = 0; i < c.n_layers; ++i) {
    LayerOff& o = m->L[i];
    const std::string p = "encoder.layers." + std::to_string(i) + ".";
    o.wqkv = m->add(p + "attention.w_q.weight", {D, D}, cur);
    m->add(p + "attention.w_k.weight", {D, D}, cur, false);
    m->add(p + "attention.w_v.weight", {D, D}, cur, false);
    o.bqkv = m->add(p + "attention.w_q.bias", {D}, cur);
    m->add(p + "attention.w_k.bias", {D}, cur, false);
    m->add(p + "attention.w_v.bias", {D}, cur, false);
    o.wo = m->add(p + "attention.w_concat.weight", {D, D}, cur);
    o.bo = m->add(p + "attention.w_concat.bias", {D}, cur);
    o.g1 = m->add(p + "norm1.gamma", {D}, cur);
    o.be1 = m->add(p + "norm1.beta", {D}, cur);
    o.w1 = m->add(p + "ffn.linear1.weight", {F, D}, cur);
    o.b1 = m->add(p + "ffn.linear1.bias", {F}, cur);
    o.w2 = m->add(p + "ffn.linear2.weight", {D, F}, cur);
    o.b2 = m->add(p + "ffn.linear2.bias", {D}, cur);
    o.g2 = m->add(p + "norm2.gamma", {D}, cur);
    o.be2 = m->add(p + "norm2.beta", {D}, cur);
    cur = align_up(cur, 64);
    o.end = cur;
  }
  m->head_begin = cur;
  m->hln_g = m->hln_b = 0;
  if (m->head_ln) {
    m->hln_g = m->add("mlp_head.0.weight", {D}, cur);
    m->hln_b = m->add("mlp_head.0.bias", {D}, cur);
    m->head_w = m->add("mlp_head.1.weight", {K, D}, cur);
    m->head_b = m->add("mlp_head.1.bias", {K}, cur);
  } else {
    m->head_w = m->add("mlp_head.weight", {K, D}, cur);
    m->head_b = m->add("mlp_head.bias", {K}, cur);
  }
  m->nparam = align_up(cur, 64);

  size_t sb = 0;
  m->sh_flat = sb; sb = align_up(sb + m->nparam * 2, 256);
  m->sh_embw = sb; sb = align_up(sb + (size_t)D * m->Ppad * 2, 256);
  for (auto& o : m->L) {
    o.t_wqkv = sb; sb = align_up(sb + (size_t)3 * D * D * 2, 256);
    o.t_wo = sb; sb = align_up(sb + (size_t)D * D * 2, 256);
    o.t_w1 = sb; sb = align_up(sb + (size_t)F * D * 2, 256);
    o.t_w2 = sb; sb = align_up(sb + (size_t)D * F * 2, 256);
  }
  for (auto& o : m->L) {
    auto push = [&](size_t src, size_t dst, int rows, int cols) {
      TransDesc d;
      d.src_off = src; d.dst_off = dst; d.rows = rows; d.cols = cols; d.tile0 = m->ttiles; d.tiles_x = (cols + 31) / 32;
      m->ttiles += d.tiles_x * ((rows + 31) / 32);
      m->ttab.push_back(d);
    };
    push(o.wqkv, o.t_wqkv, 3 * D, D);
    push(o.wo, o.t_wo, D, D);
    push(o.w1, o.t_w1, F, D);
    push(o.w2, o.t_w2, D, F);
  }
  m->sh_table = sb; sb = align_up(sb + m->ttab.size() * sizeof(TransDesc) + 64, 256);
  m->shadow_bytes = sb;
  *out = m;
  return IQ_OK;
}

extern "C" void iq_model_destroy(iq_model_t* m) {
  if (!m) return;
  delete m;
}
extern "C" const char* iq_model_last_error(const iq_model_t* m) { return m ? m->err.c_str() : "null model"; }
extern "C" int iq_model_tokens(const iq_model_t* m) { return m ? m->S : 0; }
extern "C" size_t iq_model_param_floats(const iq_model_t* m) { return m ? m->nparam : 0; }
extern "C" int iq_model_param_entries(const iq_model_t* m) { return m ? (int)m->entries.size() : 0; }
extern "C" int iq_model_param_entry(const iq_model_t* m, int i, char* name, int name_cap, size_t* offset, int* ndim,
                                    int* dims) {
  if (!m || i < 0 || i >= (int)m->entries.size() || !name || name_cap <= 0 || !offset || !ndim || !dims) return IQ_ERR_ARG;
  const Entry& e = m->entries[i];
  snprintf(name, (size_t)name_cap, "%s", e.name.c_str());
  *offset = e.off;
  *ndim = e.ndim;
  for (int k = 0; k < 4; ++k) dims[k] = e.dims[k];
  return IQ_OK;
}
extern "C" size_t iq_model_shadow_bytes(const iq_model_t* m) { return m ? m->shadow_bytes : 0; }
extern "C" size_t iq_model_workspace_bytes(const iq_model_t* m, int batch, int training) {
  (void)training;
  if (!m || batch <= 0) return 0;
  return plan_ws(m, batch).total;
}

extern "C" int iq_model_bind(iq_model_t* m, float* params, float* grads, const float* pe, void* shadow) {
  if (!m) return IQ_ERR_ARG;
  if (!params || !pe || !shadow) return fail(m, IQ_ERR_ARG, "bind: params, pe and shadow are required");
  if (((uintptr_t)params | (uintptr_t)grads | (uintptr_t)shadow) & 255) return fail(m, IQ_ERR_ARG, "bind: buffers must be 256 B aligned");
  m->params = params; m->grads = grads; m->pe = pe; m->shadow = (unsigned char*)shadow;
  if (m->table_uploaded_to != shadow && !m->ttab.empty()) {
    if (hipMemcpy(m->shadow + m->sh_table, m->ttab.data(), m->ttab.size() * sizeof(TransDesc), hipMemcpyHostToDevice) != hipSuccess)
      return fail(m, IQ_ERR_LAUNCH, "bind: uploading the transpose table failed");
    m->table_uploaded_to = shadow;
  }
  return IQ_OK;
}

extern "C" int iq_model_bind_step_counter(iq_model_t* m, uint32_t* counter) {
  if (!m) return IQ_ERR_ARG;
  if ((uintptr_t)counter & 3) return fail(m, IQ_ERR_ARG, "bind_step_counter: counter must be 4 B aligned");
  m->step_ctr = counter;
  return IQ_OK;
}

static int refresh_impl(iq_model_t* m, bool cast_flat, iq_stream_t stream) {
  if (!m || !m->params || !m->shadow) return fail(m, IQ_ERR_ARG, "refresh_shadow: model not bound");
  hipStream_t st = (hipStream_t)stream;
  const int D = m->c.d_model;
  if (cast_flat) IQ_TRY(iq_cast_bf16(m->params, m->shadow + m->sh_flat, m->nparam, stream), "cast params");
  IQ_PROF(IQ_FAM_MISC, st);
  cast_pad_kernel<<<blocks_for((size_t)D * m->Ppad), 256, 0, st>>>(m->params + m->emb_w, (bf16*)(m->shadow + m->sh_embw), D,
                                                                  m->P, m->Ppad);
  if (m->ttiles > 0)
    transpose_table_kernel<<<m->ttiles, 256, 0, st>>>(m->params, m->shadow, (const TransDesc*)(m->shadow + m->sh_table),
                                                     (int)m->ttab.size());
  return iq_launch_status();
}

extern "C" int iq_model_refresh_shadow(iq_model_t* m, iq_stream_t stream) { return refresh_impl(m, true, stream); }
extern "C" int iq_model_refresh_transposed(iq_model_t* m, iq_stream_t stream) { return refresh_impl(m, false, stream); }

extern "C" int iq_model_forward(iq_model_t* m, const float* src, int batch, void* workspace, size_t ws_bytes,
                                int training, uint64_t seed, uint32_t step, float* enc_out, float* logits,
                                iq_stream_t stream) {
  if (!m) return IQ_ERR_ARG;
  if (!m->params || !m->shadow || !m->pe) return fail(m, IQ_ERR_ARG, "forward: model not bound");
  if (!src || !workspace || batch <= 0) return fail(m, IQ_ERR_ARG, "forward: bad arguments");
  if ((uintptr_t)workspace & 255) return fail(m, IQ_ERR_ARG, "forward: workspace must be 256 B aligned");
  const WsPlan w = plan_ws(m, batch);
  if (ws_bytes < w.total) return fail(m, IQ_ERR_ARG, "forward: workspace too small");
  hipStream_t st = (hipStream_t)stream;
  unsigned char* ws = (unsigned char*)workspace;
  const iq_model_cfg_t& c = m->c;
  const int D = c.d_model, F = c.ffn_hidden, S = m->S, H = c.n_head, B = batch;
  const int M = B * S, MT = B * m->tok;
  const Route route = layer_route(M, S, D, F);
  const bool tr = training != 0 && c.drop_prob > 0.f;
  uint32_t* step_dev = m->step_ctr ? m->step_ctr : (uint32_t*)(ws + w.step_ctr);
  m->last_tr = tr;
  m->last_train_fwd = true;
  if (tr) {
    set_u32_kernel<<<1, 64, 0, st>>>(step_dev, step, step == 0xFFFFFFFFu ? 1 : 0);
    m->last_seed = seed;
  }
  const float* P = m->params;
  m->fwd_ws = nullptr;

  if (c.kind == 0) IQ_TRY(iq_patchify(src, ws + w.patches, 0, B, c.in_channels, c.img_h, c.img_w, c.patch, m->Ppad, stream), "patchify");
  else IQ_TRY(iq_patchify(src, ws + w.patches, 1, B, c.in_channels, c.seq_length, 0, c.conv_k, m->Ppad, stream), "patchify");
  const iq_dropout_t d0 = site(m, seed, step_dev, 0, tr);
  if (m->has_cls) IQ_TRY(iq_cls_rows(P + m->cls, m->pe, ws + w.x0, B, S, D, &d0, stream), "cls rows");
  {
    iq_epilogue_t e;
    memset(&e, 0, sizeof(e));
    e.bias = P + m->emb_b; e.pe = m->pe; e.tok = m->tok; e.seq = S; e.cls_off = m->has_cls; e.drop = d0;
    IQ_TRY(iq_gemm_bf16_nt(ws + w.patches, m->Ppad, m->shadow + m->sh_embw, m->Ppad, ws + w.x0, D, MT, D, m->Ppad, &e, stream),
           "embedding GEMM");
  }
  const unsigned char* x = ws + w.x0;
  bool qkv_done = false;
  for (int l = 0; l < c.n_layers; ++l) {
    const LayerOff& o = m->L[l];
    const WsPlan::L& a = w.layers[l];
    iq_epilogue_t e;
    if (!qkv_done) {
      memset(&e, 0, sizeof(e));
      e.bias = P + o.bqkv;
      IQ_TRY(iq_gemm_bf16_nt(x, D, m->sh(o.wqkv), D, ws + a.qkv, 3 * D, M, 3 * D, D, &e, stream), "qkv GEMM");
    }
    qkv_done = false;
    IQ_TRY(iq_attn_fwd(ws + a.qkv, ws + a.att, (float*)(ws + a.lse), B, S, H, m->dh, stream), "attention fwd");
    const iq_dropout_t dr1 = site(m, seed, step_dev, 1 + 3 * l, tr);
    const iq_dropout_t drh = site(m, seed, step_dev, 2 + 3 * l, tr);
    const iq_dropout_t dr2 = site(m, seed, step_dev, 3 + 3 * l, tr);
    if (route.chain) {
      const bool next = l + 1 < c.n_layers;
      IQ_TRY(iq_attn_out_ffn_chain_fwd(ws + a.att, m->sh(o.wo), P + o.bo, &dr1, x, P + o.g1, P + o.be1, ws + a.z1, ws + a.x1,
                                       (float*)(ws + a.mean1), (float*)(ws + a.rstd1), m->sh(o.w1), P + o.b1, &drh, ws + a.hid,
                                       m->sh(o.w2), P + o.b2, &dr2, P + o.g2, P + o.be2, 1e-12f, ws + a.z2, ws + a.x2,
                                       (float*)(ws + a.mean2), (float*)(ws + a.rstd2), ws + a.gate,
                                       next ? m->sh(m->L[l + 1].wqkv) : nullptr, next ? P + m->L[l + 1].bqkv : nullptr,
                                       next ? ws + w.layers[l + 1].qkv : nullptr, B, S, D, F, stream),
             "out-proj + norm1 + ffn chain + norm2 (+ next q,k,v)");
      qkv_done = next;
      x = ws + a.x2;
      continue;
    }
    if (use_fused_ln(D, D)) {
      IQ_TRY(iq_gemm_bf16_ln(ws + a.att, D, m->sh(o.wo), D, P + o.bo, x, D, &dr1, P + o.g1, P + o.be1, 1e-12f, ws + a.z1,
                             ws + a.x1, (float*)(ws + a.mean1), (float*)(ws + a.rstd1), M, D, D, stream), "out-proj GEMM + norm1");
    } else {
      memset(&e, 0, sizeof(e));
      e.bias = P + o.bo; e.drop = dr1; e.residual = x; e.ldr = D;
      IQ_TRY(iq_gemm_bf16_nt(ws + a.att, D, m->sh(o.wo), D, ws + a.z1, D, M, D, D, &e, stream), "out-proj GEMM");
      IQ_TRY(iq_ln_fwd(ws + a.z1, P + o.g1, P + o.be1, ws + a.x1, (float*)(ws + a.mean1), (float*)(ws + a.rstd1), M, D, 1e-12f, stream), "norm1");
    }
    memset(&e, 0, sizeof(e));
    e.bias = P + o.b1; e.relu = 1; e.drop = drh;
    IQ_TRY(iq_gemm_bf16_nt(ws + a.x1, D, m->sh(o.w1), D, ws + a.hid, F, M, F, D, &e, stream), "ffn1 GEMM");
    if (use_fused_ln(D, F)) {
      IQ_TRY(iq_gemm_bf16_ln(ws + a.hid, F, m->sh(o.w2), F, P + o.b2, ws + a.x1, D, &dr2, P + o.g2, P + o.be2, 1e-12f,
                             ws + a.z2, ws + a.x2, (float*)(ws + a.mean2), (float*)(ws + a.rstd2), M, D, F, stream), "ffn2 GEMM + norm2");
    } else {
      memset(&e, 0, sizeof(e));
      e.bias = P + o.b2; e.drop = dr2; e.residual = ws + a.x1; e.ldr = D;
      IQ_TRY(iq_gemm_bf16_nt(ws + a.hid, F, m->sh(o.w2), F, ws + a.z2, D, M, D, F, &e, stream), "ffn2 GEMM");
      IQ_TRY(iq_ln_fwd(ws + a.z2, P + o.g2, P + o.be2, ws + a.x2, (float*)(ws + a.mean2), (float*)(ws + a.rstd2), M, D, 1e-12f, stream), "norm2");
    }
    x = ws + a.x2;
  }
  if (logits) {
    IQ_TRY(iq_head_fwd(x, m->head_ln ? P + m->hln_g : nullptr, m->head_ln ? P + m->hln_b : nullptr, P + m->head_w,
                       P + m->head_b, (float*)(ws + w.head_feat), (float*)(ws + w.head_stat), logits, B, S, D,
                       c.num_classes, m->pool, stream), "head");
  }
  if (enc_out) bf16_to_f32_kernel<<<blocks_for((size_t)M * D / 8), 256, 0, st>>>((const bf16*)x, enc_out, (size_t)M * D / 8);
  const int rc = iq_launch_status();
  if (rc == IQ_OK) { m->fwd_ws = workspace; m->fwd_batch = batch; }
  return rc;
}

static int maps_check(iq_model_t* m, const void* workspace, size_t ws_bytes, int batch, const char* what, WsPlan* w) {
  if (!workspace || batch <= 0) return fail(m, IQ_ERR_ARG, std::string(what) + ": bad arguments");
  if (!m->fwd_ws) return fail(m, IQ_ERR_ARG, std::string(what) + ": no forward has run in a workspace");
  if (m->fwd_ws != workspace) return fail(m, IQ_ERR_ARG, std::string(what) + ": the last forward ran in another workspace");
  if (m->fwd_batch != batch)
    return fail(m, IQ_ERR_ARG, std::string(what) + ": the last forward in this workspace had batch " + std::to_string(m->fwd_batch) +
                                   ", not " + std::to_string(batch));
  *w = plan_ws(m, batch);
  if (ws_bytes < w->total) return fail(m, IQ_ERR_ARG, std::string(what) + ": workspace too small");
  return IQ_OK;
}

extern "C" int iq_model_attention(iq_model_t* m, const void* workspace, size_t ws_bytes, int batch, int layer, int rows,
                                  int heads, float* out, long out_bstride, iq_stream_t stream) {
  if (!m) return IQ_ERR_ARG;
  WsPlan w;
  const int rc = maps_check(m, workspace, ws_bytes, batch, "attention", &w);
  if (rc != IQ_OK) return rc;
  if (layer < 0 || layer >= m->c.n_layers) return fail(m, IQ_ERR_ARG, "attention: layer index out of range");
  if (rows < 0 || rows > 2 || heads < 0 || heads > 1) return fail(m, IQ_ERR_ARG, "attention: rows must be 0, 1 or 2 and heads 0 or 1");
  if (!out) return fail(m, IQ_ERR_ARG, "attention: out is NULL");
  const int S = m->S, H = m->c.n_head;
  if (out_bstride < (long)(heads ? 1 : H) * S * (rows == 0 ? S : 1)) return fail(m, IQ_ERR_ARG, "attention: out_bstride too small");
  const unsigned char* ws = (const unsigned char*)workspace;
  const WsPlan::L& a = w.layers[layer];
  IQ_TRY(iq_attn_probs(ws + a.qkv, (const float*)(ws + a.lse), out, out_bstride, batch, S, H, m->dh, rows, heads, stream),
         "attention probabilities");
  return IQ_OK;
}

extern "C" int iq_model_attention_rollout(iq_model_t* m, const void* workspace, size_t ws_bytes, int batch, float alpha,
                                          float* out, iq_stream_t stream) {
  if (!m) return IQ_ERR_ARG;
  WsPlan w;
  const int rc = maps_check(m, workspace, ws_bytes, batch, "attention rollout", &w);
  if (rc != IQ_OK) return rc;
  if (!(alpha >= 0.f && alpha <= 1.f)) return fail(m, IQ_ERR_ARG, "attention rollout: alpha must be in [0, 1]");
  if (!out) return fail(m, IQ_ERR_ARG, "attention rollout: out is NULL");
  const unsigned char* ws = (const unsigned char*)workspace;
  const int L = m->c.n_layers;
  const long qs = L > 1 ? (long)(w.layers[1].qkv - w.layers[0].qkv) : 0, ls = L > 1 ? (long)(w.layers[1].lse - w.layers[0].lse) : 0;
  for (int l = 0; l < L; ++l)
    if ((long)(w.layers[l].qkv - w.layers[0].qkv) != l * qs || (long)(w.layers[l].lse - w.layers[0].lse) != l * ls)
      return fail(m, IQ_ERR_UNSUPPORTED, "attention rollout: workspace layers are not evenly spaced");
  const size_t q0 = L ? w.layers[0].qkv : 0, l0 = L ? w.layers[0].lse : 0;
  IQ_TRY(attn_rollout_launch(ws + q0, qs, ws + l0, ls, L, out, batch, m->S, m->c.n_head, m->dh, m->has_cls, alpha,
                             (hipStream_t)stream),
         "attention rollout");
  return IQ_OK;
}

extern "C" int iq_model_grad_range(const iq_model_t* m, int stage_hi, int stage_lo, size_t* off, size_t* len) {
  if (!m || !off || !len) return IQ_ERR_ARG;
  const int Lr = m->c.n_layers;
  if (stage_lo < 0 || stage_hi > Lr + 1 || stage_lo > stage_hi) return IQ_ERR_ARG;
  auto begin = [&](int s) { return s == 0 ? (size_t)0 : (s <= Lr ? (s == 1 ? m->emb_end : m->L[s - 2].end) : m->head_begin); };
  auto end = [&](int s) { return s == 0 ? m->emb_end : (s <= Lr ? m->L[s - 1].end : m->nparam); };
  *off = begin(stage_lo);
  *len = end(stage_hi) - *off;
  return IQ_OK;
}

static int backward_impl(iq_model_t* m, const float* dlogits, const float* denc, int batch, void* workspace, size_t ws_bytes,
                         int accumulate, int stage_hi, int stage_lo, bool pgrads, iq_stream_t stream,
                         const RelHook* rh = nullptr) {
  if (!m->params || (pgrads && !m->grads) || !m->shadow) return fail(m, IQ_ERR_ARG, "backward: model not bound (grads required)");
  if (!workspace || batch <= 0) return fail(m, IQ_ERR_ARG, "backward: bad arguments");
  const iq_model_cfg_t& c = m->c;
  const int Lr = c.n_layers;
  if (stage_lo < 0 || stage_hi > Lr + 1 || stage_lo > stage_hi) return fail(m, IQ_ERR_ARG, "backward: bad stage range");
  const WsPlan w = plan_ws(m, batch);
  if (ws_bytes < w.total) return fail(m, IQ_ERR_ARG, "backward: workspace too small");
  hipStream_t st = (hipStream_t)stream;
  unsigned char* ws = (unsigned char*)workspace;
  const int D = c.d_model, F = c.ffn_hidden, S = m->S, H = c.n_head, B = batch, K = c.num_classes;
  const int M = B * S, MT = B * m->tok;
  const bool tr = m->last_tr;
  const uint32_t* step_dev = m->step_ctr ? m->step_ctr : (const uint32_t*)(ws + w.step_ctr);
  const float* P = m->params;
  float* G = m->grads;
  float* wws = (float*)(ws + w.wgrad_ws);
  const float dscale = tr ? dropout_scale(c.drop_prob) : 1.f;

  if (stage_hi == Lr + 1) {
    if (!dlogits && !denc) return fail(m, IQ_ERR_ARG, "backward: dlogits or denc required at the head stage");
    if (dlogits && !pgrads) {
      IQ_TRY(head_bwd_dx_launch(dlogits, (const float*)(ws + w.head_feat), (const float*)(ws + w.head_stat),
                                m->head_ln ? P + m->hln_g : nullptr, P + m->head_w, ws + w.gA, B, S, D, K, m->pool, st), "head bwd (dx)");
    } else if (dlogits) {
      IQ_TRY(iq_head_bwd(dlogits, (const float*)(ws + w.head_feat), (const float*)(ws + w.head_stat),
                         m->head_ln ? P + m->hln_g : nullptr, m->head_ln ? P + m->hln_b : nullptr, P + m->head_w,
                         G + m->head_w, G + m->head_b, m->head_ln ? G + m->hln_g : nullptr,
                         m->head_ln ? G + m->hln_b : nullptr, ws + w.gA, B, S, D, K, m->pool, accumulate, stream), "head bwd");
    } else if (!accumulate && pgrads) {
      (void)hipMemsetAsync(G + m->head_begin, 0, (m->nparam - m->head_begin) * sizeof(float), st);
    }
    if (denc) f32_into_bf16_kernel<<<blocks_for((size_t)M * D / 8), 256, 0, st>>>(denc, (bf16*)(ws + w.gA), (size_t)M * D / 8, dlogits ? 1 : 0);
  }
  const bool fuse1 = iq_gemm_lnbwd_supported(D, F) != 0, fuse2 = iq_gemm_lnbwd_supported(D, 3 * D) != 0;
  const Route route = layer_route(M, S, D, F);
  const bool chain = fuse1 && m->last_train_fwd && route.chain;
  bool deferred = false;
  for (int sidx = (stage_hi > Lr ? Lr : stage_hi); sidx >= 1 && sidx >= stage_lo; --sidx) {
    const int l = sidx - 1;
    const LayerOff& o = m->L[l];
    const WsPlan::L& a = w.layers[l];
    const unsigned char* xin = l == 0 ? ws + w.x0 : ws + w.layers[l - 1].x2;
    unsigned char *gZ = ws + w.gZ, *gY = ws + w.gY, *gZ1 = ws + w.gZ1, *gY1 = ws + w.gY1;
    unsigned char *gH = ws + w.gH, *gQKV = ws + w.gQKV;
    iq_epilogue_t e;
    float* lp2 = (float*)(ws + w.ln_part[0]);
    float* lp1 = (float*)(ws + w.ln_part[1]);
    const bool norm2_here = l == Lr - 1 || !fuse2;
    if (norm2_here) {
      const iq_dropout_t dr2 = m->bwd_site(3 + 3 * l, step_dev, tr);
      IQ_TRY(iq_ln_bwd(ws + w.gA, ws + a.z2, (const float*)(ws + a.mean2), (const float*)(ws + a.rstd2), P + o.g2,
                       gZ, gY, &dr2, nullptr, nullptr, lp2, accumulate, M, D, stream), "norm2 bwd");
    }
    const unsigned char* dO2 = tr ? gY : gZ;
    const unsigned char* dAo = tr ? gY1 : gZ1;
    const iq_wgrad_problem_t wg[4] = {
        {dO2, D, ws + a.hid, F, G + o.w2, G + o.b2, D, F},
        {gH, F, ws + a.x1, D, G + o.w1, G + o.b1, F, D},
        {dAo, D, ws + a.att, D, G + o.wo, G + o.bo, D, D},
        {gQKV, 3 * D, xin, D, G + o.wqkv, G + o.bqkv, 3 * D, D}};
    const int rows2 = norm2_here ? iq_ln_bwd_partial_rows(M, D) : deferred ? iq_ffn_chain_bwd_partial_rows(M) : iq_gemm_lnbwd_partial_rows(M);
    const int rows1 = chain ? iq_ffn_chain_bwd_partial_rows(M) : fuse1 ? iq_gemm_lnbwd_partial_rows(M) : iq_ln_bwd_partial_rows(M, D);
    const iq_reduce_seg_t lnseg[4] = {{lp2, rows2, 2L * D, G + o.g2, D}, {lp2 + D, rows2, 2L * D, G + o.be2, D},
                                      {lp1, rows1, 2L * D, G + o.g1, D}, {lp1 + D, rows1, 2L * D, G + o.be1, D}};
    const iq_dropout_t dr1 = m->bwd_site(1 + 3 * l, step_dev, tr);
    if (chain && deferred) {
      const LayerOff& ou = m->L[l + 1];
      const iq_dropout_t dr2b = m->bwd_site(3 + 3 * l, step_dev, tr);
      IQ_TRY(iq_qkv_dgrad_ffn_chain_bwd(gQKV, m->sht(ou.t_wqkv), gZ1, ws + a.z2, (const float*)(ws + a.mean2), (const float*)(ws + a.rstd2),
                                        P + o.g2, &dr2b, gZ, gY, lp2, m->sht(o.t_w2), ws + a.gate, dscale, gH, m->sht(o.t_w1), gZ, ws + a.z1,
                                        (const float*)(ws + a.mean1), (const float*)(ws + a.rstd1), P + o.g1, &dr1, gZ1, gY1, lp1,
                                        m->sht(o.t_wo), ws + w.gAtt, B, S, D, F, stream),
             "qkv dgrad of the layer above + norm2 bwd + ffn chain bwd + norm1 bwd + out-proj dgrad");
    } else if (chain) {
      IQ_TRY(iq_ffn_chain_bwd(dO2, m->sht(o.t_w2), ws + a.gate, dscale, gH, m->sht(o.t_w1), gZ, ws + a.z1, (const float*)(ws + a.mean1),
                              (const float*)(ws + a.rstd1), P + o.g1, &dr1, gZ1, gY1, lp1, m->sht(o.t_wo), ws + w.gAtt, B, S, D, F, stream),
             "ffn chain bwd + norm1 bwd + out-proj dgrad");
    } else {
      memset(&e, 0, sizeof(e));
      e.gate = ws + a.hid; e.ldg = F; e.gate_scale = dscale;
      IQ_TRY(iq_gemm_bf16_nt(dO2, D, m->sht(o.t_w2), D, gH, F, M, F, D, &e, stream), "ffn2 dgrad");
      if (fuse1) {
        IQ_TRY(iq_gemm_bf16_lnbwd(gH, F, m->sht(o.t_w1), F, gZ, D, ws + a.z1, (const float*)(ws + a.mean1),
                                  (const float*)(ws + a.rstd1), P + o.g1, &dr1, gZ1, gY1, lp1, M, D, F, stream), "ffn1 dgrad + norm1 bwd");
      } else {
        memset(&e, 0, sizeof(e));
        e.residual = gZ; e.ldr = D;
        IQ_TRY(iq_gemm_bf16_nt(gH, F, m->sht(o.t_w1), F, ws + w.gB, D, M, D, F, &e, stream), "ffn1 dgrad");
        IQ_TRY(iq_ln_bwd(ws + w.gB, ws + a.z1, (const float*)(ws + a.mean1), (const float*)(ws + a.rstd1), P + o.g1,
                         gZ1, gY1, &dr1, nullptr, nullptr, lp1, accumulate, M, D, stream), "norm1 bwd");
      }
    }
    if (!chain) IQ_TRY(iq_gemm_bf16_nt(dAo, D, m->sht(o.t_wo), D, ws + w.gAtt, D, M, D, D, nullptr, stream), "out-proj dgrad");
    if (rh) {
      const float* lse = (const float*)(ws + a.lse);
      if (rh->maps && rh->maps[l])
        IQ_TRY(iq_attn_grad_probs(ws + a.qkv, lse, ws + w.gAtt, rh->maps[l], rh->bstride, B, S, H, m->dh, rh->rows, rh->heads,
                                  rh->positive, stream), "gradient-weighted attention map");
      if (rh->rel) {
        const int i = Lr - 1 - l;
        IQ_TRY(attn_relevance_step_launch(ws + a.qkv, lse, ws + w.gAtt, i ? rh->r[(i - 1) & 1] : nullptr, l ? rh->r[i & 1] : rh->rel,
                                          B, S, H, m->dh, i ? 0 : m->has_cls ? 1 : 2, st), "relevance step");
      }
      if (l == 0) break;
    }
    IQ_TRY(iq_attn_bwd(ws + a.qkv, ws + a.att, ws + w.gAtt, (const float*)(ws + a.lse), gQKV, B, S, H, m->dh, stream), "attention bwd");
    if (pgrads) IQ_TRY(iq_gemm_bf16_wgrad_grouped(wg, 4, M, wws, w.wgrad_ws_bytes, accumulate, 0, lnseg, 4, stream), "layer weight gradients");
    deferred = l > 0 && fuse2 && chain && route.chain_takes_qkv_dgrad && sidx - 1 >= stage_lo;
    if (deferred) continue;
    if (l > 0 && fuse2) {
      const LayerOff& ob = m->L[l - 1];
      const WsPlan::L& ab = w.layers[l - 1];
      const iq_dropout_t dr2b = m->bwd_site(3 + 3 * (l - 1), step_dev, tr);
      IQ_TRY(iq_gemm_bf16_lnbwd(gQKV, 3 * D, m->sht(o.t_wqkv), 3 * D, gZ1, D, ws + ab.z2, (const float*)(ws + ab.mean2),
                                (const float*)(ws + ab.rstd2), P + ob.g2, &dr2b, gZ, gY, lp2, M, D, 3 * D, stream),
             "qkv dgrad + norm2 bwd of the layer below");
    } else {
      memset(&e, 0, sizeof(e));
      e.residual = gZ1; e.ldr = D;
      IQ_TRY(iq_gemm_bf16_nt(gQKV, 3 * D, m->sht(o.t_wqkv), 3 * D, ws + w.gA, D, M, D, 3 * D, &e, stream), "qkv dgrad");
    }
  }
  if (stage_lo == 0) {
    const iq_dropout_t dr0 = m->bwd_site(0, step_dev, tr);
    if (!pgrads) {
      IQ_TRY(embed_bwd_gather_launch(ws + w.gA, ws + w.demb, B, S, m->tok, D, m->has_cls, &dr0, st), "embedding bwd gather");
      return iq_launch_status();
    }
    IQ_TRY(iq_embed_bwd_gather(ws + w.gA, ws + w.demb, m->has_cls ? G + m->cls : nullptr, B, S, m->tok, D, m->has_cls,
                               &dr0, accumulate, stream), "embedding bwd gather");
    if (m->Ppad == m->P) {
      IQ_TRY(iq_gemm_bf16_wgrad(ws + w.demb, D, ws + w.patches, m->Ppad, G + m->emb_w, G + m->emb_b, MT, D, m->Ppad, wws,
                                w.wgrad_ws_bytes, accumulate, stream), "embedding wgrad");
    } else {
      float* scratch = (float*)(ws + w.embw_scratch);
      if (accumulate) (void)hipMemsetAsync(scratch, 0, (size_t)D * m->Ppad * sizeof(float), st);
      IQ_TRY(iq_gemm_bf16_wgrad(ws + w.demb, D, ws + w.patches, m->Ppad, scratch, G + m->emb_b, MT, D, m->Ppad, wws,
                                w.wgrad_ws_bytes, accumulate, stream), "embedding wgrad");
      unpad_kernel<<<blocks_for((size_t)D * m->P), 256, 0, st>>>(scratch, G + m->emb_w, D, m->P, m->Ppad, accumulate);
    }
  }
  return iq_launch_status();
}

extern "C" int iq_model_backward(iq_model_t* m, const float* dlogits, const float* denc, int batch, void* workspace,
                                 size_t ws_bytes, int accumulate, int stage_hi, int stage_lo, iq_stream_t stream) {
  if (!m) return IQ_ERR_ARG;
  return backward_impl(m, dlogits, denc, batch, workspace, ws_bytes, accumulate, stage_hi, stage_lo, true, stream);
}

extern "C" int iq_model_backward_input(iq_model_t* m, const float* dlogits, const float* denc, int batch, void* workspace,
                                       size_t ws_bytes, float* dsrc, int flags, iq_stream_t stream) {
  if (!m) return IQ_ERR_ARG;
  if (flags & ~IQ_BWD_PARAM_GRADS) return fail(m, IQ_ERR_ARG, "backward_input: unknown flags");
  if (!dsrc) return fail(m, IQ_ERR_ARG, "backward_input: dsrc is NULL");
  if (!dlogits && !denc) return fail(m, IQ_ERR_ARG, "backward_input: dlogits or denc required");
  const bool pgrads = (flags & IQ_BWD_PARAM_GRADS) != 0;
  if (!m->params || !m->shadow || !m->pe) return fail(m, IQ_ERR_ARG, "backward_input: model not bound");
  if (pgrads && !m->grads) return fail(m, IQ_ERR_ARG, "backward_input: IQ_BWD_PARAM_GRADS needs a bound gradient buffer");
  WsPlan w;
  const int rc = maps_check(m, workspace, ws_bytes, batch, "backward_input", &w);
  if (rc != IQ_OK) return rc;
  const int rb = backward_impl(m, dlogits, denc, batch, workspace, ws_bytes, 0, m->c.n_layers + 1, 0, pgrads, stream);
  if (rb != IQ_OK) return rb;
  const iq_model_cfg_t& c = m->c;
  unsigned char* ws = (unsigned char*)workspace;
  const int kind = c.kind, H = kind == 0 ? c.img_h : c.seq_length, W = kind == 0 ? c.img_w : 0, p = kind == 0 ? c.patch : c.conv_k;
  IQ_TRY(iq_embed_dgrad(ws + w.demb, m->shadow + m->sh_embw, m->Ppad, dsrc, kind, batch, c.in_channels, H, W, p, c.d_model, stream),
         "embedding data gradient");
  return IQ_OK;
}

extern "C" int iq_model_attention_relevance(iq_model_t* m, const float* dlogits, int batch, void* workspace, size_t ws_bytes,
                                            float* rel, float* const* maps, int rows, int heads, int positive, long out_bstride,
                                            iq_stream_t stream) {
  if (!m) return IQ_ERR_ARG;
  if (!m->params || !m->shadow || !m->pe) return fail(m, IQ_ERR_ARG, "attention relevance: model not bound");
  if (!dlogits) return fail(m, IQ_ERR_ARG, "attention relevance: dlogits is NULL");
  WsPlan w;
  const int rc = maps_check(m, workspace, ws_bytes, batch, "attention relevance", &w);
  if (rc != IQ_OK) return rc;
  if (rows < 0 || rows > 2 || heads < 0 || heads > 1)
    return fail(m, IQ_ERR_ARG, "attention relevance: rows must be 0, 1 or 2 and heads 0 or 1");
  if (positive < 0 || positive > 1) return fail(m, IQ_ERR_ARG, "attention relevance: positive must be 0 or 1");
  const int L = m->c.n_layers, S = m->S, H = m->c.n_head;
  bool any_map = false;
  for (int l = 0; maps && l < L; ++l) any_map = any_map || maps[l];
  if (!rel && !any_map) return fail(m, IQ_ERR_ARG, "attention relevance: rel and every map are NULL");
  if (any_map && out_bstride < (long)(heads ? 1 : H) * S * (rows == 0 ? S : 1))
    return fail(m, IQ_ERR_ARG, "attention relevance: out_bstride too small");
  RelHook h;
  h.maps = maps; h.rows = rows; h.heads = heads; h.positive = positive; h.bstride = out_bstride; h.rel = rel;
  h.r[0] = (float*)((unsigned char*)workspace + w.demb);
  h.r[1] = h.r[0] + (size_t)batch * S;
  if (2 * (size_t)batch * S * sizeof(float) > (size_t)batch * m->tok * m->c.d_model * 2)
    return fail(m, IQ_ERR_UNSUPPORTED, "attention relevance: no room for the relevance vectors");
  if (L == 0) {
    if (rel) rel_start_kernel<<<blocks_for((size_t)batch * S), 256, 0, (hipStream_t)stream>>>(rel, batch * S, S, m->has_cls);
    return iq_launch_status() == IQ_OK ? IQ_OK : fail(m, IQ_ERR_LAUNCH, "attention relevance: start vector launch failed");
  }
  return backward_impl(m, dlogits, nullptr, batch, workspace, ws_bytes, 0, L + 1, 1, false, stream, &h);
}
```

Baseline: 53330 frames/s.

## Run per-layer wgrad slab reduce on spare workgroups of the qkv-dgrad LN-bwd GEMM

Splits the grouped weight-gradient launch so its split-K slab reduction is deferred into a job descriptor. The job is then executed by extra workgroups appended to the following fused qkv-dgrad + norm2-backward GEMM launch, using CU slots the GEMM tiles leave idle. This removes one reduce kernel launch per layer and overlaps the reduction with the GEMM. To avoid a race, the LN partial buffer is now triple-buffered by layer parity. The cost is extra workspace, some occupancy-query complexity, and possible contention between the reduce and GEMM workgroups.

```diff
diff --git a/include/iqvit.h b/include/iqvit.h
--- a/include/iqvit.h
+++ b/include/iqvit.h
@@ -102,6 +102,31 @@
 int iq_gemm_bf16_wgrad_grouped(const iq_wgrad_problem_t* probs, int nprob, int M, float* ws, size_t ws_bytes,
                                int accumulate, int max_workgroups, const iq_reduce_seg_t* extra, int nextra,
                                iq_stream_t stream);
+
+#define IQ_REDUCE_JOB_SEGS 12
+typedef struct iq_reduce_job_seg {
+  const float* partials;
+  float* out;
+  int64_t n;
+  int64_t stride;
+  int rows;
+  int blk0;
+  int tall;
+} iq_reduce_job_seg_t;
+typedef struct iq_reduce_job {
+  iq_reduce_job_seg_t seg[IQ_REDUCE_JOB_SEGS];
+  int nseg;
+  int nblk;
+  int accumulate;
+} iq_reduce_job_t;
+int iq_gemm_bf16_wgrad_grouped_deferred(const iq_wgrad_problem_t* probs, int nprob, int M, float* ws, size_t ws_bytes,
+                                        int accumulate, int max_workgroups, const iq_reduce_seg_t* extra, int nextra,
+                                        iq_reduce_job_t* job, iq_stream_t stream);
+int iq_reduce_job_run(const iq_reduce_job_t* job, iq_stream_t stream);
+int iq_gemm_lnbwd_ride_workgroups(int M, int D, int K, int job_blocks);
+int iq_gemm_bf16_lnbwd_ride(const void* A, int lda, const void* Wt, int ldw, const void* residual, int ldr, const void* z,
+                            const float* mean, const float* rstd, const float* gamma, const iq_dropout_t* drop, void* dz,
+                            void* dy, float* partial, int M, int D, int K, const iq_reduce_job_t* job, iq_stream_t stream);
 
 int iq_attn_supported(int S, int dh);
 int iq_attn_fwd(const void* qkv, void* out, float* lse, int B, int S, int H, int dh, iq_stream_t stream);
diff --git a/vit-vs-raw-iq_amd/_native.py b/vit-vs-raw-iq_amd/_native.py
--- a/vit-vs-raw-iq_amd/_native.py
+++ b/vit-vs-raw-iq_amd/_native.py
@@ -74,6 +74,15 @@
 class ReduceSeg(C.Structure):
     _fields_ = [("partials", C.c_void_p), ("rows", C.c_int), ("row_stride", C.c_int64), ("out", C.c_void_p),
                 ("n", C.c_int64)]
+
+
+class ReduceJobSeg(C.Structure):
+    _fields_ = [("partials", C.c_void_p), ("out", C.c_void_p), ("n", C.c_int64), ("stride", C.c_int64), ("rows", C.c_int),
+                ("blk0", C.c_int), ("tall", C.c_int)]
+
+
+class ReduceJob(C.Structure):
+    _fields_ = [("seg", ReduceJobSeg * 12), ("nseg", C.c_int), ("nblk", C.c_int), ("accumulate", C.c_int)]
 
 
 class ModelCfg(C.Structure):
@@ -113,6 +122,11 @@
     "iq_gemm_bf16_wgrad": (_I, [_P, _I, _P, _I, _P, _P, _I, _I, _I, _P, _Z, _I, _P]),
     "iq_wgrad_grouped_ws_bytes": (_Z, [_P, _I, _I, _I]),
     "iq_gemm_bf16_wgrad_grouped": (_I, [_P, _I, _I, _P, _Z, _I, _I, _P, _I, _P]),
+    "iq_gemm_bf16_wgrad_grouped_deferred": (_I, [_P, _I, _I, _P, _Z, _I, _I, _P, _I, C.POINTER(ReduceJob), _P]),
+    "iq_reduce_job_run": (_I, [C.POINTER(ReduceJob), _P]),
+    "iq_gemm_bf16_lnbwd_ride": (_I, [_P, _I, _P, _I, _P, _I, _P, _P, _P, _P, C.POINTER(Dropout), _P, _P, _P, _I, _I, _I,
+                                     C.POINTER(ReduceJob), _P]),
+    "iq_gemm_lnbwd_ride_workgroups": (_I, [_I, _I, _I, _I]),
     "iq_attn_supported": (_I, [_I, _I]),
     "iq_attn_fwd": (_I, [_P, _P, _P, _I, _I, _I, _I, _P]),
     "iq_attn_bwd": (_I, [_P, _P, _P, _P, _P, _I, _I, _I, _I, _P]),
diff --git a/vit-vs-raw-iq_amd/csrc/gemm_lnbwd.hip b/vit-vs-raw-iq_amd/csrc/gemm_lnbwd.hip
--- a/vit-vs-raw-iq_amd/csrc/gemm_lnbwd.hip
+++ b/vit-vs-raw-iq_amd/csrc/gemm_lnbwd.hip
@@ -4,10 +4,14 @@
 #include "gemm_ring.h"
 #include "iqvit.h"
 #include "prof.h"
+#include "wgrad_reduce.h"
 
 namespace {
 
 constexpr int LB_THREADS = 256;
+static_assert(LB_THREADS == RED_THREADS, "a reduce-role workgroup is a virtual block of the slab reduce");
+
+constexpr int RIDE_ROWS = 8;
 
 struct LnBwdParams {
   const bf16* A; const bf16* B; const bf16* residual;
@@ -19,7 +23,7 @@
 };
 
 template <int BMT, int BN>
-__global__ __launch_bounds__(LB_THREADS, 2) void gemm_lnbwd_kernel(const LnBwdParams p) {
+__global__ __launch_bounds__(LB_THREADS, 2) void gemm_lnbwd_kernel(const LnBwdParams p, const RedGroup job) {
   using Ring = RingShape<BMT, BN>;
   constexpr int BK2 = Ring::BK2, NS = Ring::NS, STAGE_BYTES = Ring::STAGE_BYTES, WN = Ring::WN, NT = Ring::NT, NP = NT / 2, MT = Ring::MT;
   constexpr int A_LD = Ring::A_LD, B_LD = Ring::B_LD, PER_STAGE = Ring::PER_STAGE, NRS = Ring::NRS;
@@ -27,6 +31,14 @@
   constexpr int N = BN;
   static_assert(NRS >= 2, "tile shape");
   extern __shared__ __attribute__((aligned(16))) unsigned char smem[];
+  static_assert(RED_THREADS * 16 <= NS * STAGE_BYTES, "the reduce role's LDS fits in the ring");
+  {
+    const int tiles = (p.M + BMT - 1) / BMT;
+    if ((int)blockIdx.x >= tiles) {
+      red_walk<RIDE_ROWS>(job, (int)blockIdx.x - tiles, (int)gridDim.x - tiles, reinterpret_cast<f32x4*>(smem));
+      return;
+    }
+  }
 
   const int tid = threadIdx.x, lane = tid & 63, wave = tid >> 6;
   const int wm = wave >> 1, wn = wave & 1;
@@ -275,11 +287,39 @@
 }
 
 template <int BMT, int BN>
-int launch(const LnBwdParams& p, hipStream_t st) {
-  const size_t lds = RingShape<BMT, BN>::BYTES + (2 * BMT + BN) * sizeof(float);
+constexpr size_t lnbwd_lds() { return RingShape<BMT, BN>::BYTES + (2 * BMT + BN) * sizeof(float); }
+
+template <int BMT, int BN>
+int lnbwd_slots() {
+  static const int slots = [] {
+    auto k = gemm_lnbwd_kernel<BMT, BN>;
+    const size_t lds = lnbwd_lds<BMT, BN>();
+    if (lds > 48 * 1024) (void)hipFuncSetAttribute((const void*)k, hipFuncAttributeMaxDynamicSharedMemorySize, (int)lds);
+    int dev = 0, cus = 0, per_cu = 0;
+    if (hipGetDevice(&dev) != hipSuccess || hipDeviceGetAttribute(&cus, hipDeviceAttributeMultiprocessorCount, dev) != hipSuccess ||
+        hipOccupancyMaxActiveBlocksPerMultiprocessor(&per_cu, k, LB_THREADS, lds) != hipSuccess) {
+      (void)hipGetLastError();
+      return 0;
+    }
+    return per_cu * cus;
+  }();
+  return slots;
+}
+
+constexpr int RIDE_MIN_WGS = 64;
+template <int BMT, int BN>
+int lnbwd_ride_wgs(int M, int nblk) {
+  const int tiles = (M + BMT - 1) / BMT, spare = lnbwd_slots<BMT, BN>() - tiles;
+  if (nblk <= 0 || spare < RIDE_MIN_WGS) return 0;
+  return spare < nblk ? spare : nblk;
+}
+
+template <int BMT, int BN>
+int launch(const LnBwdParams& p, const RedGroup& job, int ride_wgs, hipStream_t st) {
+  const size_t lds = lnbwd_lds<BMT, BN>();
   auto k = gemm_lnbwd_kernel<BMT, BN>;
   if (lds > 48 * 1024) (void)hipFuncSetAttribute((const void*)k, hipFuncAttributeMaxDynamicSharedMemorySize, (int)lds);
-  k<<<(p.M + BMT - 1) / BMT, LB_THREADS, lds, st>>>(p);
+  k<<<(p.M + BMT - 1) / BMT + ride_wgs, LB_THREADS, lds, st>>>(p, job);
   return iq_launch_status();
 }
 
@@ -294,11 +334,13 @@
   return (M + r - 1) / r;
 }
 
-extern "C" int iq_gemm_bf16_lnbwd(const void* A, int lda, const void* Wt, int ldw, const void* residual, int ldr,
-                                  const void* z, const float* mean, const float* rstd, const float* gamma,
-                                  const iq_dropout_t* drop, void* dz, void* dy, float* partial, int M, int D, int K,
-                                  iq_stream_t stream) {
-  if (M <= 0) return IQ_OK;
+extern "C" int iq_gemm_bf16_lnbwd_ride(const void* A, int lda, const void* Wt, int ldw, const void* residual, int ldr,
+                                       const void* z, const float* mean, const float* rstd, const float* gamma,
+                                       const iq_dropout_t* drop, void* dz, void* dy, float* partial, int M, int D, int K,
+                                       const iq_reduce_job_t* job, iq_stream_t stream) {
+  const bool have_job = job && job->nblk > 0;
+  if (have_job && (job->nseg <= 0 || job->nseg > IQ_REDUCE_JOB_SEGS)) return IQ_ERR_ARG;
+  if (M <= 0) return have_job ? iq_reduce_job_run(job, stream) : IQ_OK;
   if (!A || !Wt || !residual || !z || !mean || !rstd || !gamma || !dz || !partial) return IQ_ERR_ARG;
   if (!iq_gemm_lnbwd_supported(D, K) || (lda % 8) || (ldw % 8) || (ldr % 8)) return IQ_ERR_UNSUPPORTED;
   if (((uintptr_t)A | (uintptr_t)Wt | (uintptr_t)residual | (uintptr_t)z | (uintptr_t)dz | (uintptr_t)dy | (uintptr_t)gamma) % 16)
@@ -310,9 +352,35 @@
   p.dZ = (bf16*)dz; p.dY = (bf16*)dy; p.partial = partial;
   if (!dropout_unpack(drop, &p.drop_on, &p.rng, &p.thresh, &p.dscale) || (p.drop_on && !dy)) return IQ_ERR_ARG;
   hipStream_t st = (hipStream_t)stream;
+  const bool b64 = lnbwd_block_rows(M) == 64;
+  RedGroup none = {};
+  int wgs = 0;
+  if (have_job) {
+    const int nblk = job->nblk;
+    wgs = b64 ? (D == 192 ? lnbwd_ride_wgs<64, 192>(M, nblk) : lnbwd_ride_wgs<64, 128>(M, nblk))
+              : (D == 192 ? lnbwd_ride_wgs<128, 192>(M, nblk) : lnbwd_ride_wgs<128, 128>(M, nblk));
+    if (wgs == 0) {
+      const int rc = iq_reduce_job_run(job, stream);
+      if (rc != IQ_OK) return rc;
+    }
+  }
+  const RedGroup& rj = wgs > 0 ? *job : none;
   IQ_PROF(IQ_FAM_GEMM_NT, st);
   IQ_PROF_K(2.0 * ((double)M * K + (double)D * K + (double)M * D * (3 + (p.drop_on ? 1 : 0))) + 8.0 * M, 2.0 * (double)M * D * K,
             "gemm_lnbwd_kernel<%d, %d>", lnbwd_block_rows(M), D);
-  if (lnbwd_block_rows(M) == 64) return D == 192 ? launch<64, 192>(p, st) : launch<64, 128>(p, st);
-  return D == 192 ? launch<128, 192>(p, st) : launch<128, 128>(p, st);
-}
+  if (b64) return D == 192 ? launch<64, 192>(p, rj, wgs, st) : launch<64, 128>(p, rj, wgs, st);
+  return D == 192 ? launch<128, 192>(p, rj, wgs, st) : launch<128, 128>(p, rj, wgs, st);
+}
+
+extern "C" int iq_gemm_lnbwd_ride_workgroups(int M, int D, int K, int job_blocks) {
+  if (M <= 0 || !iq_gemm_lnbwd_supported(D, K)) return 0;
+  if (lnbwd_block_rows(M) == 64) return D == 192 ? lnbwd_ride_wgs<64, 192>(M, job_blocks) : lnbwd_ride_wgs<64, 128>(M, job_blocks);
+  return D == 192 ? lnbwd_ride_wgs<128, 192>(M, job_blocks) : lnbwd_ride_wgs<128, 128>(M, job_blocks);
+}
+
+extern "C" int iq_gemm_bf16_lnbwd(const void* A, int lda, const void* Wt, int ldw, const void* residual, int ldr,
+                                  const void* z, const float* mean, const float* rstd, const float* gamma,
+                                  const iq_dropout_t* drop, void* dz, void* dy, float* partial, int M, int D, int K,
+                                  iq_stream_t stream) {
+  return iq_gemm_bf16_lnbwd_ride(A, lda, Wt, ldw, residual, ldr, z, mean, rstd, gamma, drop, dz, dy, partial, M, D, K, nullptr, stream);
+}
diff --git a/vit-vs-raw-iq_amd/csrc/gemm_wgrad.hip b/vit-vs-raw-iq_amd/csrc/gemm_wgrad.hip
--- a/vit-vs-raw-iq_amd/csrc/gemm_wgrad.hip
+++ b/vit-vs-raw-iq_amd/csrc/gemm_wgrad.hip
@@ -5,6 +5,7 @@
 #include "prof.h"
 
 #include "gemm_wgrad_big.h"
+#include "wgrad_reduce.h"
 
 namespace {
 
@@ -350,46 +351,10 @@
   else pw_body<64, 64>(g, p, tile, split, smem);
 }
 
-constexpr int RED_MAXX = 4;
-struct RedSeg { const float* slab; float* out; long n, stride; int rows, blk0, tall; };
-struct RedGroup { RedSeg s[2 * PW_MAXP + RED_MAXX]; int nseg, accumulate; };
-
-inline int red_blocks(long n, int tall) { return (int)((n + (tall ? 63 : 255)) / (tall ? 64 : 256)); }
-
-__global__ __launch_bounds__(256) void wgrad_reduce_kernel(const RedGroup g) {
-  __shared__ f32x4 part[256];
-  RedSeg sg = g.s[0];
-#pragma unroll
-  for (int i = 1; i < 2 * PW_MAXP + RED_MAXX; ++i)
-    if (i < g.nseg && (int)blockIdx.x >= g.s[i].blk0) sg = g.s[i];
-  const float* __restrict__ slab = sg.slab;
-  float* __restrict__ out = sg.out;
-  const long n = sg.n, stride = sg.stride;
-  const long blk = (long)blockIdx.x - sg.blk0;
-  const int rows = sg.rows, accumulate = g.accumulate;
-  const int ncol = sg.tall ? 16 : 64, nsl = 256 / ncol;
-  const int col = threadIdx.x % ncol, sl = threadIdx.x / ncol;
-  const long i = (blk * ncol + col) * 4;
-  f32x4 s = {0.f, 0.f, 0.f, 0.f};
-  if (i + 4 <= n) {
-#pragma unroll 8
-    for (int sp = sl; sp < rows; sp += nsl) s += *reinterpret_cast<const f32x4*>(slab + (long)sp * stride + i);
-  } else if (i < n) {
-    for (int sp = sl; sp < rows; sp += nsl)
-      for (int e = 0; e < 4 && i + e < n; ++e) s[e] += slab[(long)sp * stride + i + e];
-  }
-  part[sl * ncol + col] = s;
-  __syncthreads();
-  if (sl == 0 && i < n) {
-    f32x4 t = part[col];
-    for (int k = 1; k < nsl; ++k) t += part[k * ncol + col];
-    if (i + 4 <= n) {
-      f32x4* o = reinterpret_cast<f32x4*>(out + i);
-      *o = accumulate ? *o + t : t;
-    } else {
-      for (int e = 0; e < 4 && i + e < n; ++e) out[i + e] = accumulate ? out[i + e] + t[e] : t[e];
-    }
-  }
+static_assert(RED_MAXP == PW_MAXP, "a reduce job holds the segments of one group");
+__global__ __launch_bounds__(RED_THREADS) void wgrad_reduce_kernel(const RedGroup g) {
+  __shared__ f32x4 part[RED_THREADS];
+  red_block(g, (int)blockIdx.x, part);
 }
 
 struct WgradPlan { int tk, mc, tiles_n, tiles_k, splits, rows_per_split; };
@@ -459,9 +424,10 @@
 unsigned long long* g_wstamps = nullptr;
 #endif
 
-int launch_reduce(const RedGroup& rg, int nblk, hipStream_t st) {
+int launch_reduce(const RedGroup& rg, hipStream_t st) {
+  if (rg.nblk <= 0) return IQ_OK;
   IQ_PROF(IQ_FAM_WGRAD, st);
-  wgrad_reduce_kernel<<<nblk, 256, 0, st>>>(rg);
+  wgrad_reduce_kernel<<<rg.nblk, RED_THREADS, 0, st>>>(rg);
   IQ_PROF_K(0.0, 0.0, "wgrad_reduce_kernel");
   return IQ_OK;
 }
@@ -505,12 +471,13 @@
   RedGroup rg;
   memset(&rg, 0, sizeof(rg));
   const long n = (long)N * K;
-  rg.s[0] = RedSeg{q.slab, pb.dW, n, n, w.splits, 0, 0};
+  rg.seg[0] = RedSeg{q.slab, pb.dW, n, n, w.splits, 0, 0};
   int nblk = (int)((n + 255) / 256);
   rg.nseg = 1;
-  if (pb.dbias) { rg.s[1] = RedSeg{q.bslab, pb.dbias, (long)N, (long)N, w.splits, nblk, 0}; nblk += (N + 255) / 256; rg.nseg = 2; }
+  if (pb.dbias) { rg.seg[1] = RedSeg{q.bslab, pb.dbias, (long)N, (long)N, w.splits, nblk, 0}; nblk += (N + 255) / 256; rg.nseg = 2; }
   rg.accumulate = accumulate;
-  return launch_reduce(rg, nblk, st);
+  rg.nblk = nblk;
+  return launch_reduce(rg, st);
 }
 
 }
@@ -541,9 +508,25 @@
   return mx * sizeof(float);
 }
 
+extern "C" int iq_reduce_job_run(const iq_reduce_job_t* job, iq_stream_t stream) {
+  if (!job || job->nblk < 0 || job->nseg < 0 || job->nseg > IQ_REDUCE_JOB_SEGS) return IQ_ERR_ARG;
+  launch_reduce(*job, (hipStream_t)stream);
+  return iq_launch_status();
+}
+
 extern "C" int iq_gemm_bf16_wgrad_grouped(const iq_wgrad_problem_t* probs, int nprob, int M, float* ws, size_t ws_bytes,
                                           int accumulate, int max_workgroups, const iq_reduce_seg_t* extra, int nextra,
                                           iq_stream_t stream) {
+  iq_reduce_job_t job;
+  const int rc = iq_gemm_bf16_wgrad_grouped_deferred(probs, nprob, M, ws, ws_bytes, accumulate, max_workgroups, extra, nextra, &job, stream);
+  return rc != IQ_OK ? rc : iq_reduce_job_run(&job, stream);
+}
+
+extern "C" int iq_gemm_bf16_wgrad_grouped_deferred(const iq_wgrad_problem_t* probs, int nprob, int M, float* ws, size_t ws_bytes,
+                                                   int accumulate, int max_workgroups, const iq_reduce_seg_t* extra, int nextra,
+                                                   iq_reduce_job_t* job, iq_stream_t stream) {
+  if (!job) return IQ_ERR_ARG;
+  memset(job, 0, sizeof(*job));
   if (nextra < 0 || nextra > RED_MAXX || (nextra > 0 && !extra)) return IQ_ERR_ARG;
   for (int i = 0; i < nextra; ++i)
     if (!extra[i].partials || !extra[i].out || extra[i].rows <= 0 || extra[i].n <= 0 || extra[i].row_stride < extra[i].n ||
@@ -552,7 +535,7 @@
   auto add_extra = [&](RedGroup& rg, int& nblk) {
     for (int i = 0; i < nextra; ++i) {
       const int tall = extra[i].rows >= 64;
-      rg.s[rg.nseg++] = RedSeg{extra[i].partials, extra[i].out, (long)extra[i].n, (long)extra[i].row_stride, extra[i].rows, nblk, tall};
+      rg.seg[rg.nseg++] = RedSeg{extra[i].partials, extra[i].out, (long)extra[i].n, (long)extra[i].row_stride, extra[i].rows, nblk, tall};
       nblk += red_blocks(extra[i].n, tall);
     }
   };
@@ -581,16 +564,17 @@
     int nblk = 0;
     for (int i = 0; i < nprob; ++i) {
       const long n = (long)probs[i].N * probs[i].K;
-      rg.s[rg.nseg++] = RedSeg{slab[i], probs[i].dW, n, (long)pad4((size_t)n), wb.splits, nblk, 0};
+      rg.seg[rg.nseg++] = RedSeg{slab[i], probs[i].dW, n, (long)pad4((size_t)n), wb.splits, nblk, 0};
       nblk += (int)((n + 255) / 256);
       if (probs[i].dbias) {
-        rg.s[rg.nseg++] = RedSeg{bslab[i], probs[i].dbias, (long)probs[i].N, (long)pad4(probs[i].N), wb.splits, nblk, 0};
+        rg.seg[rg.nseg++] = RedSeg{bslab[i], probs[i].dbias, (long)probs[i].N, (long)pad4(probs[i].N), wb.splits, nblk, 0};
         nblk += (probs[i].N + 255) / 256;
       }
     }
     add_extra(rg, nblk);
     rg.accumulate = accumulate;
-    launch_reduce(rg, nblk, st);
+    rg.nblk = nblk;
+    *job = rg;
     return iq_launch_status();
   }
   if (!group_is_pw(probs, nprob)) {
@@ -609,7 +593,8 @@
       int nblk = 0;
       add_extra(rg, nblk);
       rg.accumulate = accumulate;
-      launch_reduce(rg, nblk, st);
+      rg.nblk = nblk;
+      *job = rg;
     }
     return iq_launch_status();
   }
@@ -635,11 +620,11 @@
     tile0 += q.tiles_n * q.tiles_k;
     const long n = (long)b.N * b.K;
     q.slab = cur; cur += (size_t)w.splits * pad4((size_t)n);
-    rg.s[rg.nseg++] = RedSeg{q.slab, b.dW, n, n, w.splits, nblk, 0};
+    rg.seg[rg.nseg++] = RedSeg{q.slab, b.dW, n, n, w.splits, nblk, 0};
     nblk += (int)((n + 255) / 256);
     if (b.dbias) {
       q.bslab = cur; cur += (size_t)w.splits * pad4(b.N);
-      rg.s[rg.nseg++] = RedSeg{q.bslab, b.dbias, (long)b.N, (long)b.N, w.splits, nblk, 0};
+      rg.seg[rg.nseg++] = RedSeg{q.bslab, b.dbias, (long)b.N, (long)b.N, w.splits, nblk, 0};
       nblk += (b.N + 255) / 256;
     }
   }
@@ -652,7 +637,8 @@
     wgrad_pw_kernel<<<w.ntile * w.splits, PW_THREADS, lds_pw, st>>>(g);
     IQ_PROF_K(wbytes, wflops, "wgrad_pw_kernel");
   }
-  launch_reduce(rg, nblk, st);
+  rg.nblk = nblk;
+  *job = rg;
   return iq_launch_status();
 }
 
diff --git a/vit-vs-raw-iq_amd/csrc/model.hip b/vit-vs-raw-iq_amd/csrc/model.hip
--- a/vit-vs-raw-iq_amd/csrc/model.hip
+++ b/vit-vs-raw-iq_amd/csrc/model.hip
@@ -35,7 +35,7 @@
   size_t step_ctr, patches, x0, head_feat, head_stat;
   struct L { size_t qkv, att, lse, z1, mean1, rstd1, x1, hid, gate, z2, mean2, rstd2, x2; };
   std::vector<L> layers;
-  size_t gA, gB, gAtt, demb, wgrad_ws, wgrad_ws_bytes, ln_part[2], embw_scratch;
+  size_t gA, gB, gAtt, demb, wgrad_ws, wgrad_ws_bytes, ln_part[3], embw_scratch;
   size_t gZ, gY, gZ1, gY1, gH, gQKV;
   size_t total;
 };
@@ -234,7 +234,7 @@
   if ((size_t)iq_ffn_chain_bwd_partial_rows((int)M) > ln_rows_fused) ln_rows_fused = (size_t)iq_ffn_chain_bwd_partial_rows((int)M);
   ln_rows_fused *= 2 * D * sizeof(float);
   const size_t ln_bytes = ln_rows_fused > iq_ln_bwd_ws_bytes((int)D) ? ln_rows_fused : iq_ln_bwd_ws_bytes((int)D);
-  for (int k = 0; k < 2; ++k) w.ln_part[k] = take(ln_bytes);
+  for (int k = 0; k < 3; ++k) w.ln_part[k] = take(ln_bytes);
   w.embw_scratch = take((size_t)D * m->Ppad * 4 + 256);
   w.total = cur;
   return w;
@@ -649,7 +649,8 @@
     unsigned char *gZ = ws + w.gZ, *gY = ws + w.gY, *gZ1 = ws + w.gZ1, *gY1 = ws + w.gY1;
     unsigned char *gH = ws + w.gH, *gQKV = ws + w.gQKV;
     iq_epilogue_t e;
-    float* lp2 = (float*)(ws + w.ln_part[0]);
+    auto ln2_part = [&](int layer) { return (float*)(ws + w.ln_part[(layer & 1) ? 2 : 0]); };
+    float* lp2 = ln2_part(l);
     float* lp1 = (float*)(ws + w.ln_part[1]);
     const bool norm2_here = l == Lr - 1 || !fuse2;
     if (norm2_here) {
@@ -710,16 +711,24 @@
       if (l == 0) break;
     }
     IQ_TRY(iq_attn_bwd(ws + a.qkv, ws + a.att, ws + w.gAtt, (const float*)(ws + a.lse), gQKV, B, S, H, m->dh, stream), "attention bwd");
-    if (pgrads) IQ_TRY(iq_gemm_bf16_wgrad_grouped(wg, 4, M, wws, w.wgrad_ws_bytes, accumulate, 0, lnseg, 4, stream), "layer weight gradients");
     deferred = l > 0 && fuse2 && chain && route.chain_takes_qkv_dgrad && sidx - 1 >= stage_lo;
+    const bool ride = pgrads && l > 0 && fuse2 && !deferred;
+    iq_reduce_job_t job;
+    if (ride) {
+      IQ_TRY(iq_gemm_bf16_wgrad_grouped_deferred(wg, 4, M, wws, w.wgrad_ws_bytes, accumulate, 0, lnseg, 4, &job, stream),
+             "layer weight gradients (partial tiles)");
+    } else if (pgrads) {
+      IQ_TRY(iq_gemm_bf16_wgrad_grouped(wg, 4, M, wws, w.wgrad_ws_bytes, accumulate, 0, lnseg, 4, stream), "layer weight gradients");
+    }
     if (deferred) continue;
     if (l > 0 && fuse2) {
       const LayerOff& ob = m->L[l - 1];
       const WsPlan::L& ab = w.layers[l - 1];
       const iq_dropout_t dr2b = m->bwd_site(3 + 3 * (l - 1), step_dev, tr);
-      IQ_TRY(iq_gemm_bf16_lnbwd(gQKV, 3 * D, m->sht(o.t_wqkv), 3 * D, gZ1, D, ws + ab.z2, (const float*)(ws + ab.mean2),
-                                (const float*)(ws + ab.rstd2), P + ob.g2, &dr2b, gZ, gY, lp2, M, D, 3 * D, stream),
-             "qkv dgrad + norm2 bwd of the layer below");
+      IQ_TRY(iq_gemm_bf16_lnbwd_ride(gQKV, 3 * D, m->sht(o.t_wqkv), 3 * D, gZ1, D, ws + ab.z2, (const float*)(ws + ab.mean2),
+                                     (const float*)(ws + ab.rstd2), P + ob.g2, &dr2b, gZ, gY, ln2_part(l - 1), M, D, 3 * D,
+                                     ride ? &job : nullptr, stream),
+             "qkv dgrad + norm2 bwd of the layer below (+ this layer's slab reduce)");
     } else {
       memset(&e, 0, sizeof(e));
       e.residual = gZ1; e.ldr = D;
diff --git a/vit-vs-raw-iq_amd/csrc/wgrad_reduce.h b/vit-vs-raw-iq_amd/csrc/wgrad_reduce.h
--- /dev/null
+++ b/vit-vs-raw-iq_amd/csrc/wgrad_reduce.h
@@ -0,0 +1,89 @@
+#pragma once
+#include "common.h"
+
+constexpr int RED_THREADS = 256;
+constexpr int RED_MAXP = 4;
+constexpr int RED_MAXX = 4;
+static_assert(IQ_REDUCE_JOB_SEGS == 2 * RED_MAXP + RED_MAXX, "iq_reduce_job_t holds a group's segments");
+typedef iq_reduce_job_seg_t RedSeg;
+typedef iq_reduce_job_t RedGroup;
+
+inline int red_blocks(long n, int tall) { return (int)((n + (tall ? 63 : 255)) / (tall ? 64 : 256)); }
+
+struct RedLane {
+  const float* slab; float* out;
+  long n, stride, i;
+  int rows, ncol, nsl, col, sl;
+};
+__device__ __forceinline__ RedLane red_lane(const RedGroup& g, int vb) {
+  RedSeg sg = g.seg[0];
+#pragma unroll
+  for (int i = 1; i < 2 * RED_MAXP + RED_MAXX; ++i)
+    if (i < g.nseg && vb >= g.seg[i].blk0) sg = g.seg[i];
+  RedLane l;
+  l.slab = sg.partials; l.out = sg.out; l.n = sg.n; l.stride = sg.stride; l.rows = sg.rows;
+  const long blk = (long)vb - sg.blk0;
+  l.ncol = sg.tall ? 16 : 64; l.nsl = RED_THREADS / l.ncol;
+  l.col = threadIdx.x % l.ncol; l.sl = threadIdx.x / l.ncol;
+  l.i = (blk * l.ncol + l.col) * 4;
+  return l;
+}
+__device__ __forceinline__ void red_tail_sum(const RedLane& l, f32x4& s) {
+  for (int sp = l.sl; sp < l.rows; sp += l.nsl)
+    for (int e = 0; e < 4 && l.i + e < l.n; ++e) s[e] += l.slab[(long)sp * l.stride + l.i + e];
+}
+__device__ __forceinline__ void red_combine(const RedLane& l, const f32x4* part, int accumulate) {
+  if (l.sl == 0 && l.i < l.n) {
+    f32x4 t = part[l.col];
+    for (int k = 1; k < l.nsl; ++k) t += part[k * l.ncol + l.col];
+    if (l.i + 4 <= l.n) {
+      f32x4* o = reinterpret_cast<f32x4*>(l.out + l.i);
+      *o = accumulate ? *o + t : t;
+    } else {
+      for (int e = 0; e < 4 && l.i + e < l.n; ++e) l.out[l.i + e] = accumulate ? l.out[l.i + e] + t[e] : t[e];
+    }
+  }
+}
+
+__device__ __forceinline__ void red_block(const RedGroup& g, int vb, f32x4* part) {
+  const RedLane l = red_lane(g, vb);
+  const float* __restrict__ slab = l.slab;
+  f32x4 s = {0.f, 0.f, 0.f, 0.f};
+  if (l.i + 4 <= l.n) {
+#pragma unroll 8
+    for (int sp = l.sl; sp < l.rows; sp += l.nsl) s += *reinterpret_cast<const f32x4*>(slab + (long)sp * l.stride + l.i);
+  } else if (l.i < l.n) {
+    red_tail_sum(l, s);
+  }
+  part[l.sl * l.ncol + l.col] = s;
+  __syncthreads();
+  red_combine(l, part, g.accumulate);
+}
+
+template <int ROWS>
+__device__ __forceinline__ void red_walk(const RedGroup& g, int first, int step, f32x4* part) {
+  for (int vb = first; vb < g.nblk; vb += step) {
+    const RedLane l = red_lane(g, vb);
+    f32x4 s = {0.f, 0.f, 0.f, 0.f};
+    if (l.i + 4 <= l.n) {
+      for (int sp0 = l.sl; sp0 < l.rows; sp0 += ROWS * l.nsl) {
+        f32x4 v[ROWS];
+#pragma unroll
+        for (int u = 0; u < ROWS; ++u) {
+          const int sp = sp0 + u * l.nsl;
+          v[u] = f32x4{0.f, 0.f, 0.f, 0.f};
+          if (sp < l.rows) v[u] = *reinterpret_cast<const f32x4*>(l.slab + (long)sp * l.stride + l.i);
+        }
+#pragma unroll
+        for (int u = 0; u < ROWS; ++u)
+          if (sp0 + u * l.nsl < l.rows) s += v[u];
+      }
+    } else if (l.i < l.n) {
+      red_tail_sum(l, s);
+    }
+    part[l.sl * l.ncol + l.col] = s;
+    __syncthreads();
+    red_combine(l, part, g.accumulate);
+    __syncthreads();
+  }
+}
```

Measured after the change: 53930 frames/s (median of 6 runs). 1.1% higher.
